# miaoyin390/DNN-Compression-Tensor-ADMM

Measured on AMD Instinct MI355X. Metric: ADMM projection iters/sec (all layers) + per-layer SVD GFLOP/s, ResNet-50 TT ranks, higher is better.
Workload: dtype f32 (Gram, eigen-solve and its filter products accumulate in f64); 1 GPU; resnet50_tt: 34 layers, 20099072 weights, hp table tt_resnet50_hp.HyperParamsDictGeneralRatio3x; tables=1, parallelism=layer-shard x1 (latency-model partition, one scalar all-reduce per step)

## Files before the change

dnn-compression-tensor-admm_amd/csrc/abi_ops.hip:

```cpp
#include "host.h"

using namespace tadmm;

__global__ void square_copy_kernel(const double* __restrict__ in, double* __restrict__ out, int n) {
  const int i = blockIdx.x * blockDim.x + threadIdx.x;
  if (i < n) out[i] = in[i] * in[i];
}

static GemmDesc to_gemm_desc(const tadmm_gemm_desc& s) {
  GemmDesc g;
  memset(&g, 0, sizeof g);
  g.A = s.A; g.B = s.B; g.C = s.C; g.M = s.M; g.N = s.N; g.K = s.K;
  g.a_rs = s.a_rs; g.a_cs = s.a_cs; g.b_rs = s.b_rs; g.b_cs = s.b_cs; g.c_rs = s.c_rs; g.c_cs = s.c_cs;
  g.alpha = s.alpha; g.beta = s.beta; g.bias_n = s.bias_n; g.bias_m = s.bias_m;
  return g;
}

extern "C" {

int tadmm_version(void) { return 100; }

int tadmm_abi_sizes(int* layer_desc_bytes, int* gemm_desc_bytes) {
  if (layer_desc_bytes) *layer_desc_bytes = (int)sizeof(tadmm_layer_desc);
  if (gemm_desc_bytes) *gemm_desc_bytes = (int)sizeof(tadmm_gemm_desc);
// ... 260 lines not shown
  if (c->dtype == TADMM_CHAIN_F16)
    CTX_FAIL(h, TADMM_ERR_INVALID, "conv chain: binary16 is inference only (tadmm_ttconv_fused)");
  ConvChainDesc d;
  const int rc = conv_chain_shape(h, c, mode, d, nullptr);
  if (rc != TADMM_OK) return rc;
  if (r1 <= 0 || r1 > c->R1 || r2 <= 0 || r2 > c->R2)
    CTX_FAIL(h, TADMM_ERR_INVALID, "conv chain: true ranks (%d, %d) outside (0, %d] x (0, %d]", r1, r2, c->R1, c->R2);
  const bool bwd = mode == TADMM_CONV_CHAIN_BWD;
  if (!bwd && (!s1 || !s2) && c->B > 0) CTX_FAIL(h, TADMM_ERR_INVALID, "conv chain: null intermediate (H1, H2)");
  if (bwd && (s1 == nullptr) != (s2 == nullptr)) CTX_FAIL(h, TADMM_ERR_INVALID, "conv chain: dH1 and dH2 are saved together or not at all");
  if (c->B > 0 && (!c->X || !c->Y || !c->W1 || !c->W2 || !c->W3)) CTX_FAIL(h, TADMM_ERR_INVALID, "conv chain: null operand");
  const uintptr_t esz = c->dtype == TADMM_CHAIN_F32 ? 4 : 2;
  if (((uintptr_t)c->X | (uintptr_t)c->Y | (uintptr_t)s1 | (uintptr_t)s2) & (esz - 1))
    CTX_FAIL(h, TADMM_ERR_INVALID, "conv chain: misaligned operand");
  if (!conv_chain_planes_ok(c, d) || (!bwd && (((uintptr_t)c->bias) & 15)))
    CTX_FAIL(h, TADMM_ERR_INVALID, "conv chain: weight planes too small or misaligned");
  if (c->B == 0) return TADMM_OK;
  conv_chain_operands(c, d);
  d.bias = bwd ? nullptr : c->bias;
  d.S1 = bwd ? s2 : s1; d.S2 = bwd ? s1 : s2;
  d.r1t = bwd ? r2 : r1; d.r2t = bwd ? r1 : r2;
  return conv_chain_launch(h, d, c->dtype, (hipStream_t)stream_);
}

int tadmm_ttconv_fused_save(tadmm_handle h, const tadmm_conv_chain_desc* d, int r1, int r2, void* H1, void* H2, void* stream) {
  return conv_chain_train(h, d, TADMM_CONV_CHAIN_FWD, r1, r2, H1, H2, stream);
}

int tadmm_ttconv_fused_bwd(tadmm_handle h, const tadmm_conv_chain_desc* d, int r1, int r2, void* dH1, void* dH2, void* stream) {
  return conv_chain_train(h, d, TADMM_CONV_CHAIN_BWD, r1, r2, dH1, dH2, stream);
}

int tadmm_ttconv_fused_plan(const tadmm_conv_chain_desc* c, int mode, int* tile_pixels, int* tile_rows, int* halo_tiles,
                            int* tiles_per_image, size_t* lds_bytes) {
  if (!c || (mode != TADMM_CONV_CHAIN_FWD && mode != TADMM_CONV_CHAIN_BWD)) return TADMM_ERR_INVALID;
  ConvChainDesc d;
  size_t lds = 0;
  const int rc = conv_chain_shape(nullptr, c, mode, d, &lds);
  if (rc != TADMM_OK) return rc;
  if (tile_pixels) *tile_pixels = d.TM;
  if (tile_rows) *tile_rows = d.TR;
  if (halo_tiles) *halo_tiles = d.NT;
  if (tiles_per_image) *tiles_per_image = d.tiles;
  if (lds_bytes) *lds_bytes = lds;
  return TADMM_OK;
}

int tadmm_core_conv_desc_bytes(void) { return (int)sizeof(tadmm_core_conv_desc); }

int tadmm_core_conv_fwd(tadmm_handle h, const tadmm_core_conv_desc* d, void* stream_) {
  DeviceGuard device_guard(h);
  if (!h) return TADMM_ERR_INVALID;
  return launch_core_conv(h, d, 0, (hipStream_t)stream_);
}

int tadmm_core_conv_dgrad(tadmm_handle h, const tadmm_core_conv_desc* d, void* stream_) {
  DeviceGuard device_guard(h);
  if (!h) return TADMM_ERR_INVALID;
  return launch_core_conv(h, d, 1, (hipStream_t)stream_);
}

static EigGeom gram_geom(int m, int n) { return eig_geom(m, n, 256, false); }

size_t tadmm_gram_scratch_bytes(int m, int n) {
  const EigGeom st = gram_geom(m, n);
  const size_t ntp = (size_t)st.nt * (st.nt + 1) / 2;
  const size_t nblk_p = (size_t)st.ksplit * ntp;
  const size_t nblk_r = ((size_t)st.Npad * st.ld + 1023) / 1024;
  return align_up(st.ksplit * ntp * 1024 * 8, 256) + align_up(sizeof(GramDesc), 256) +
         align_up(nblk_p * sizeof(BlockRef), 256) + align_up(nblk_r * sizeof(BlockRef), 256);
}

int tadmm_gram_ld(int m, int n, int* Npad, int* ld) {
  const EigGeom st = gram_geom(m, n);
  if (Npad) *Npad = st.Npad;
  if (ld) *ld = st.ld;
  return st.N;
}

int tadmm_gram_f64(tadmm_handle h, const float* A, int m, int n, double* G, int ldg, void* scratch, size_t scratch_bytes,
                   void* stream_) {
  DeviceGuard device_guard(h);
  if (!h || !A || !G || !scratch || m <= 0 || n <= 0) return TADMM_ERR_INVALID;
  const EigGeom st = gram_geom(m, n);
  if (ldg != st.ld) CTX_FAIL(h, TADMM_ERR_INVALID, "ldg must be %d (tadmm_gram_ld)", st.ld);
  if (scratch_bytes < tadmm_gram_scratch_bytes(m, n)) CTX_FAIL(h, TADMM_ERR_WORKSPACE, "gram scratch too small");
  hipStream_t s = (hipStream_t)stream_;
  const size_t ntp = (size_t)st.nt * (st.nt + 1) / 2;
  char* base = (char*)scratch;
  size_t off = 0;
  double* partial = (double*)(base + off); off += align_up(st.ksplit * ntp * 1024 * 8, 256);
  GramDesc* gdev = (GramDesc*)(base + off); off += align_up(sizeof(GramDesc), 256);
  std::vector<BlockRef> mp, mr;
  for (int b = 0; b < (int)(st.ksplit * ntp); ++b) mp.push_back(BlockRef{0, b});
  if (st.ksplit > 1)
    for (int b = 0; b < (int)(((size_t)st.Npad * st.ld + 1023) / 1024); ++b) mr.push_back(BlockRef{0, b});
  BlockRef* mpd = (BlockRef*)(base + off); off += align_up(mp.size() * sizeof(BlockRef), 256);
  BlockRef* mrd = (BlockRef*)(base + off);
  GramDesc gd;
  memset(&gd, 0, sizeof gd);
  gd.A = A; gd.m = m; gd.n = n; gd.trans = st.trans; gd.N = st.N; gd.K = st.trans ? m : n; gd.nt = st.nt;
  gd.ksplit = st.ksplit; gd.kchunk = st.kchunk; gd.partial = partial; gd.G = G; gd.Npad = st.Npad; gd.ld = st.ld;
  HIP_OK(h, hipMemcpyAsync(gdev, &gd, sizeof gd, hipMemcpyHostToDevice, s));
  HIP_OK(h, hipMemcpyAsync(mpd, mp.data(), mp.size() * sizeof(BlockRef), hipMemcpyHostToDevice, s));
  HIP_OK(h, hipMemcpyAsync(mrd, mr.data(), mr.size() * sizeof(BlockRef), hipMemcpyHostToDevice, s));
  HIP_OK(h, hipStreamSynchronize(s));
  launch_gram_partial(gdev, mpd, (int)mp.size(), s);
  launch_gram_reduce(gdev, mrd, (int)mr.size(), s);
  HIP_OK(h, hipGetLastError());
  return TADMM_OK;
}

size_t tadmm_eigh_scratch_bytes(int N) {
  const EigGeom g = eig_geom(N, N, 64, true);
  const size_t Npad = g.Npad, ld = g.ld;
  return align_up(Npad * ld * 8, 256) + align_up(sizeof(EigDesc), 256) + 3 * align_up(Npad * sizeof(BlockRef), 256) +
         align_up(Npad * 8, 256) * 2 + align_up(Npad * 4, 256) + 1024 + align_up((Npad / 16) * 256 * 8, 256);
}

static int eigh_leading(tadmm_handle h, const double* G, int N, int r, double* evals_out, double* evecs_out,
                        void* scratch, size_t scratch_bytes, int* sweeps_out, int* route_out, void* stream_) {
  DeviceGuard device_guard(h);
  if (!h || !G || !evals_out || !evecs_out || !scratch || N <= 0 || r < 1 || r > N) return TADMM_ERR_INVALID;
  if (scratch_bytes < tadmm_eigh_scratch_bytes(N)) CTX_FAIL(h, TADMM_ERR_WORKSPACE, "eigh scratch too small");
  hipStream_t s = (hipStream_t)stream_;
  const EigGeom geo = eig_geom(N, N, 64, true);
  const int Npad = geo.Npad, ld = geo.ld;
  char* base = (char*)scratch;
  size_t off = 0;
  auto carve = [&](size_t bytes) { const size_t o = off; off += align_up(bytes, 256); return o; };
  double* XT = (double*)(base + carve((size_t)Npad * ld * 8));
  const size_t o_desc = carve(sizeof(EigDesc));
  EigDesc* edev = (EigDesc*)(base + o_desc);
  EigLayout L;
  Phase* phases[3] = {&L.tick, &L.norm, &L.ext};
  size_t o_map[3];
  for (size_t& o : o_map) o = carve(Npad * sizeof(BlockRef));
  double* lam = (double*)(base + carve((size_t)Npad * 8));
  double* sigma = (double*)(base + carve((size_t)Npad * 8));
  int32_t* order = (int32_t*)(base + carve((size_t)Npad * 4));
  double* offs = (double*)(base + off); off += 64;
  int32_t* done = (int32_t*)(base + off); off += 64;
  double* sblk = (double*)(base + off);
  HIP_OK(h, hipMemsetAsync(XT, 0, (size_t)Npad * ld * 8, s));
  HIP_OK(h, hipMemcpy2DAsync(XT, (size_t)ld * 8, G, (size_t)N * 8, (size_t)N * 8, N, hipMemcpyDeviceToDevice, s));
  std::vector<EigDesc> ev(1);
  EigDesc& e = ev[0];
  memset(&e, 0, sizeof e);
  e.XT = XT; e.N = N; e.Npad = Npad; e.ld = ld; e.nb = geo.nb; e.off = offs; e.done = done; e.lam = lam; e.order = order;
  e.sigma = sigma; e.r = r; e.mode = 2; e.out_a = nullptr; e.out_b = nullptr; e.evec_out = evecs_out;
  e.sblk = sblk;
  EigMaps maps;
  if (const int rc = eig_maps(h, L, ev, false, maps)) return rc;
  const std::vector<BlockRef>* mv[3] = {&maps.tick, &maps.norm, &maps.ext};
  HIP_OK(h, hipMemcpyAsync(edev, &e, sizeof e, hipMemcpyHostToDevice, s));
  for (int i = 0; i < 3; ++i) {
    phases[i]->desc_off = o_desc;
    phases[i]->map_off = o_map[i];
    HIP_OK(h, hipMemcpyAsync(base + o_map[i], mv[i]->data(), mv[i]->size() * sizeof(BlockRef), hipMemcpyHostToDevice, s));
  }
  HIP_OK(h, hipStreamSynchronize(s));
  const bool super = L.kernel == EigTick::SuperPairs;
  const int units = L.players[0];
  const BlockRef* m_tick = (const BlockRef*)(base + L.tick.map_off);
  const double tol = 1e-9;
  int tick = 0, gs = 0;
  bool conv = false;
  if (jacobi_small_fits(Npad) && !(getenv("TADMM_EIGH_TICK") && atoi(getenv("TADMM_EIGH_TICK")))) {
    int32_t* fast = done + 4;
    int* verdict = (int*)(done + 8);
    HIP_OK(h, hipMemsetAsync(done, 0, 64, s));
    const bool direct = eig_small_direct_on();
    if (direct) HIP_OK(h, launch_eig_small_direct(edev, 1, nullptr, fast, verdict, s));
    HIP_OK(h, launch_jacobi_small(edev, 1, Npad, tol, 60, nullptr, verdict, s, false, direct ? fast : nullptr));
    int hv[6] = {0, 0, 0, 0, 0, 0};
    HIP_OK(h, hipMemcpyAsync(hv, done + 4, sizeof hv, hipMemcpyDeviceToHost, s));
    HIP_OK(h, hipStreamSynchronize(s));
    conv = hv[5] != 0;
    gs = hv[0] ? 0 : 1;
    if (sweeps_out) *sweeps_out = gs;
    if (route_out) *route_out = hv[0] ? 0 : 1;
    if (!conv) CTX_FAIL(h, TADMM_ERR_NOCONVERGE, "small eigen-solve did not converge");
  } else {
  if (route_out) *route_out = 2;
  launch_jacobi_init(edev, 1, s);
  double hoff[3];
  int hdone = 0;
  for (; gs < 40 && !conv; ++gs) {
    for (int t = 0; t < units - 1; ++t, ++tick) {
      if (super) {
        HIP_OK(h, launch_jacobi_tick3(edev, m_tick, L.tick.nblocks, tick, tol, ld, s));
      } else {
        HIP_OK(h, launch_jacobi_tick(edev, m_tick, L.tick.nblocks, tick, tol, L.tick_lds, s));
      }
    }
    HIP_OK(h, hipMemcpyAsync(hoff, offs, 24, hipMemcpyDeviceToHost, s));
    HIP_OK(h, hipMemcpyAsync(&hdone, done, 4, hipMemcpyDeviceToHost, s));
    HIP_OK(h, hipStreamSynchronize(s));
    conv = hdone || hoff[gs & 1] < tol;
  }
  if (sweeps_out) *sweeps_out = gs;
  if (getenv("TADMM_STAMPS_DUMP")) { (void)hipStreamSynchronize(s); dump_stamps(); }
  if (!conv) CTX_FAIL(h, TADMM_ERR_NOCONVERGE, "Jacobi did not converge in 40 sweeps");
  }
  L.finalize(base, s, nullptr);
  HIP_OK(h, hipGetLastError());
  hipLaunchKernelGGL(square_copy_kernel, dim3((r + 255) / 256), dim3(256), 0, s, sigma, evals_out, r);
  HIP_OK(h, hipGetLastError());
  return TADMM_OK;
}

int tadmm_eigh_f64(tadmm_handle h, const double* G, int N, double* evals_out, double* evecs_out, void* scratch,
                   size_t scratch_bytes, int* sweeps_out, void* stream_) {
  return eigh_leading(h, G, N, N, evals_out, evecs_out, scratch, scratch_bytes, sweeps_out, nullptr, stream_);
}

int tadmm_eigh_partial_f64(tadmm_handle h, const double* G, int N, int r, double* evals_out, double* evecs_out,
                           void* scratch, size_t scratch_bytes, int* route_out, void* stream_) {
  return eigh_leading(h, G, N, r, evals_out, evecs_out, scratch, scratch_bytes, nullptr, route_out, stream_);
}

size_t tadmm_dgemm_scratch_bytes(int M, int N) {
  return align_up(sizeof(DgemmDesc), 256) + align_up((size_t)(M / 32) * (N / 32) * sizeof(BlockRef), 256);
}

int tadmm_dgemm_f64(tadmm_handle h, const double* A, const double* B, double* C, int M, int N, int K, int lda, int ldb,
                    int ldc, int b_transposed, void* scratch, size_t scratch_bytes, void* stream_) {
  DeviceGuard device_guard(h);
  if (!h || !A || !B || !C || !scratch) return TADMM_ERR_INVALID;
  if (M <= 0 || N <= 0 || K <= 0 || M % 32 || N % 32 || K % 16 || (lda & 1) || (ldb & 1) || (ldc & 1))
    CTX_FAIL(h, TADMM_ERR_INVALID, "tadmm_dgemm_f64: M, N multiples of 32, K of 16, even leading dimensions");
  if (scratch_bytes < tadmm_dgemm_scratch_bytes(M, N)) CTX_FAIL(h, TADMM_ERR_WORKSPACE, "dgemm scratch too small");
  hipStream_t s = (hipStream_t)stream_;
  DgemmDesc g;
  memset(&g, 0, sizeof g);
  g.A = A; g.B = B; g.C = C; g.selA = g.selB = g.selC = g.selP = g.selQ = -1;
  g.M = M; g.N = N; g.K = K; g.lda = lda; g.ldb = ldb; g.ldc = ldc; g.tiles_m = M / 32; g.tiles_n = N / 32;
  std::vector<BlockRef> map;
  for (int b = 0; b < g.tiles_m * g.tiles_n; ++b) map.push_back(BlockRef{0, b});
  DgemmDesc* gd = (DgemmDesc*)scratch;
  BlockRef* md = (BlockRef*)((char*)scratch + align_up(sizeof(DgemmDesc), 256));
  HIP_OK(h, hipMemcpyAsync(gd, &g, sizeof g, hipMemcpyHostToDevice, s));
  HIP_OK(h, hipMemcpyAsync(md, map.data(), map.size() * sizeof(BlockRef), hipMemcpyHostToDevice, s));
  HIP_OK(h, hipStreamSynchronize(s));
  if (b_transposed && K % 32 == 0 && !getenv("TADMM_DGEMM_OLD")) {
    std::vector<BlockRef> m64;
    for (int b = 0; b < ((M + 63) / 64) * ((N + 63) / 64); ++b) m64.push_back(BlockRef{0, b});
    HIP_OK(h, hipMemcpyAsync(md, m64.data(), m64.size() * sizeof(BlockRef), hipMemcpyHostToDevice, s));
    HIP_OK(h, hipStreamSynchronize(s));
    launch_dgemm_nt64(gd, md, (int)m64.size(), s);
  } else {
    launch_dgemm(gd, md, (int)map.size(), b_transposed != 0, s);
  }
  HIP_OK(h, hipGetLastError());
  return TADMM_OK;
}

size_t tadmm_dgemm3_scratch_bytes(int M, int N) {
  const size_t planes = (size_t)3 * (N / 16) * (N / 32) * 512 * 2;
  return align_up(sizeof(DgemmDesc), 256) + align_up(sizeof(GPlaneDesc), 256) + align_up(planes, 256) +
         2 * align_up(((size_t)(M / 32) * ((N + 63) / 64) + (size_t)(N / 16) * (N / 32) / 4 + 8) * sizeof(BlockRef), 256);
}

int tadmm_dgemm3_f64(tadmm_handle h, const double* A, const double* Gm, double* C, int M, int N, int lda, int ldg, int ldc,
                     int repeats, void* scratch, size_t scratch_bytes, void* stream_) {
  DeviceGuard device_guard(h);
  if (!h || !A || !Gm || !C || !scratch) return TADMM_ERR_INVALID;
  if (M <= 0 || N <= 0 || M % 32 || N % 32 || lda < N || ldg < N || ldc < N || (lda & 1) || (ldg & 1) || (ldc & 1))
    CTX_FAIL(h, TADMM_ERR_INVALID, "tadmm_dgemm3_f64: M, N multiples of 32, even leading dimensions >= N");
  if (scratch_bytes < tadmm_dgemm3_scratch_bytes(M, N)) CTX_FAIL(h, TADMM_ERR_WORKSPACE, "dgemm3 scratch too small");
  hipStream_t s = (hipStream_t)stream_;
  char* base = (char*)scratch;
  size_t off = 0;
  auto take = [&](size_t b) { size_t o = off; off += align_up(b, 256); return o; };
  const size_t o_g = take(sizeof(DgemmDesc)), o_p = take(sizeof(GPlaneDesc));
  const int nt = N / 16, ks = N / 32;
  const int64_t plane = (int64_t)nt * ks * 512;
  const size_t o_planes = take((size_t)3 * plane * 2);
  std::vector<BlockRef> m_gp, m_fast;
  for (int b = 0; b < (nt * ks + 3) / 4; ++b) m_gp.push_back(BlockRef{0, b});
  const int tn = (N + 63) / 64;
  for (int b = 0; b < (M / 32) * tn; ++b) m_fast.push_back(BlockRef{0, b});
  xcd_by_key(m_fast, [&](const BlockRef& b) { return b.local % tn; });
  const size_t o_mgp = take(m_gp.size() * sizeof(BlockRef)), o_mf = take(m_fast.size() * sizeof(BlockRef));
  GPlaneDesc gd;
  memset(&gd, 0, sizeof gd);
  gd.Gm = Gm; gd.ldg = ldg; gd.nt = nt; gd.ks = ks; gd.out = (uint16_t*)(base + o_planes); gd.plane = plane;
  DgemmDesc g;
  memset(&g, 0, sizeof g);
  g.A = A; g.C = C; g.selA = g.selB = g.selC = g.selP = g.selQ = -1;
  g.M = M; g.N = N; g.K = N; g.lda = lda; g.ldb = ldg; g.ldc = ldc; g.tiles_m = M / 32; g.tiles_n = N / 32;
  g.Gp = (const uint16_t*)(base + o_planes); g.g_plane = plane;
  HIP_OK(h, hipMemcpyAsync(base + o_g, &g, sizeof g, hipMemcpyHostToDevice, s));
  HIP_OK(h, hipMemcpyAsync(base + o_p, &gd, sizeof gd, hipMemcpyHostToDevice, s));
  HIP_OK(h, hipMemcpyAsync(base + o_mgp, m_gp.data(), m_gp.size() * sizeof(BlockRef), hipMemcpyHostToDevice, s));
  HIP_OK(h, hipMemcpyAsync(base + o_mf, m_fast.data(), m_fast.size() * sizeof(BlockRef), hipMemcpyHostToDevice, s));
  HIP_OK(h, hipStreamSynchronize(s));
  launch_gplanes((const GPlaneDesc*)(base + o_p), (const BlockRef*)(base + o_mgp), (int)m_gp.size(), s);
  for (int i = 0; i < std::max(1, repeats); ++i)
    launch_dgemm3((const DgemmDesc*)(base + o_g), (const BlockRef*)(base + o_mf), (int)m_fast.size(), s);
  HIP_OK(h, hipGetLastError());
  return TADMM_OK;
}

size_t tadmm_cholqr_scratch_bytes(int n, int ncols) {
  return align_up(sizeof(DgemmDesc), 256) + align_up(sizeof(CholDesc), 256) + 2 * align_up((size_t)n * n * 8, 256) +
         align_up((size_t)n * 16 * 8, 256) + align_up((size_t)(n / 32) * (n / 32) * sizeof(BlockRef), 256) +
         align_up((size_t)(ncols / kCholStrip) * sizeof(BlockRef), 256) + 256;
}

int tadmm_cholqr_f64(tadmm_handle h, double* YT, int n, int ncols, int ldy, void* scratch, size_t scratch_bytes,
                     int* bad_out_host, void* stream_) {
  DeviceGuard device_guard(h);
  if (!h || !YT || !scratch || !bad_out_host) return TADMM_ERR_INVALID;
  if (n <= 0 || n > 256 || n % 32 || ncols <= 0 || ncols % 64 || ldy < ncols || (ldy & 1))
    CTX_FAIL(h, TADMM_ERR_INVALID, "tadmm_cholqr_f64: n multiple of 32 (<= 256), ncols multiple of 64, ldy >= ncols even");
  if (scratch_bytes < tadmm_cholqr_scratch_bytes(n, ncols)) CTX_FAIL(h, TADMM_ERR_WORKSPACE, "cholqr scratch too small");
  hipStream_t s = (hipStream_t)stream_;
  char* base = (char*)scratch;
  size_t off = 0;
  DgemmDesc* gd = (DgemmDesc*)(base + off); off += align_up(sizeof(DgemmDesc), 256);
  CholDesc* cd = (CholDesc*)(base + off); off += align_up(sizeof(CholDesc), 256);
  double* Cm = (double*)(base + off); off += align_up((size_t)n * n * 8, 256);
  double* Rm = (double*)(base + off); off += align_up((size_t)n * n * 8, 256);
  double* Wd = (double*)(base + off); off += align_up((size_t)n * 16 * 8, 256);
  BlockRef* mg = (BlockRef*)(base + off); off += align_up((size_t)(n / 32) * (n / 32) * sizeof(BlockRef), 256);
  BlockRef* ms = (BlockRef*)(base + off); off += align_up((size_t)(ncols / kCholStrip) * sizeof(BlockRef), 256);
  int32_t* bad = (int32_t*)(base + off);
  DgemmDesc g;
  memset(&g, 0, sizeof g);
  g.A = YT; g.B = YT; g.C = Cm; g.selA = g.selB = g.selC = g.selP = g.selQ = -1;
  g.M = n; g.N = n; g.K = ncols; g.lda = ldy; g.ldb = ldy; g.ldc = n; g.tiles_m = n / 32; g.tiles_n = n / 32;
  CholDesc c;
  memset(&c, 0, sizeof c);
  c.C = Cm; c.ldc = n; c.n = n; c.R = Rm; c.ldr = n; c.Wd = Wd;
  c.ring[0] = YT; c.ring[1] = YT; c.ring[2] = YT; c.rot = nullptr; c.sel = 0; c.ldy = ldy; c.ncols = ncols; c.bad = bad;
  std::vector<BlockRef> vg, vs;
  for (int b = 0; b < g.tiles_m * g.tiles_n; ++b) vg.push_back(BlockRef{0, b});
  for (int b = 0; b < ncols / kCholStrip; ++b) vs.push_back(BlockRef{0, b});
  HIP_OK(h, hipMemsetAsync(bad, 0, 4, s));
  HIP_OK(h, hipMemcpyAsync(gd, &g, sizeof g, hipMemcpyHostToDevice, s));
  HIP_OK(h, hipMemcpyAsync(cd, &c, sizeof c, hipMemcpyHostToDevice, s));
  HIP_OK(h, hipMemcpyAsync(mg, vg.data(), vg.size() * sizeof(BlockRef), hipMemcpyHostToDevice, s));
  HIP_OK(h, hipMemcpyAsync(ms, vs.data(), vs.size() * sizeof(BlockRef), hipMemcpyHostToDevice, s));
// ... 96 lines not shown
```

dnn-compression-tensor-admm_amd/csrc/common.h:

```cpp
#pragma once
#include <hip/hip_runtime.h>
#include <stdint.h>
#include <stddef.h>
#include "../../include/tadmm.h"

namespace tadmm {

constexpr int kWave = 64;

struct BlockRef { int32_t prob; int32_t local; };

struct SweepDesc {
  const float* W; float* U; float* Z;
  float* T0;
  const float* Zmat;
  int32_t O, I, K2;
  int32_t ichunk;
  int32_t nchunk;
  int64_t numel;
  int32_t blk_begin;
  int32_t nblk;
};

void launch_unfold(const SweepDesc* descs_dev, const BlockRef* map_dev, int nblocks, int use_u, hipStream_t s);
void launch_fold_update(const SweepDesc* descs_dev, const BlockRef* map_dev, int nblocks, int update_u,
                        double* resid_partial_dev, hipStream_t s);
void launch_resid_reduce(const SweepDesc* descs_dev, int nlayers, const double* resid_partial_dev,
                         double* resid_sq_dev, hipStream_t s, const int32_t* out_index = nullptr);

struct GramDesc {
  const float* A;
  int32_t m, n;
  int32_t trans;
  int32_t N, K;
  int32_t nt;
  int32_t ksplit, kchunk;
  double* partial;
  double* G;
  int32_t Npad, ld;
};
void launch_gram_partial(const GramDesc* descs_dev, const BlockRef* map_dev, int nblocks, hipStream_t s,
                         const int32_t* skip = nullptr);
void launch_gram_reduce(const GramDesc* descs_dev, const BlockRef* map_dev, int nblocks, hipStream_t s,
                        const int32_t* skip = nullptr);

constexpr int kJB = 8;
struct EigDesc {
  double* XT;
  int32_t N, Npad, ld, nb;
  double* off;
  int32_t* done;
  double* lam;
  int32_t* order;
  double* sigma;
  int32_t r;
  int32_t mode;
  float* out_a;
  float* out_b;
  double* evec_out;
  double* sblk;
  int32_t ldo;
  double* warm;
  int32_t* warm_ok;
  double* scratch;
  int32_t period;
};
void launch_jacobi_init(const EigDesc* descs_dev, int nprob, hipStream_t s, const int32_t* skip = nullptr,
                        double* prev_dev = nullptr);
void launch_jacobi_conv(const EigDesc* descs_dev, int nprob, int tick, double tol, bool super, double* prev_dev,
                        int* verdict_pinned, hipStream_t s);
constexpr int kJacobiMaxN = 8160;
bool jacobi_size_supported(int n);
size_t jacobi_tick_stream_lds_bytes();
size_t jacobi_tick_lds_bytes(int ld_max);
hipError_t launch_jacobi_tick(const EigDesc* descs_dev, const BlockRef* map_dev, int nblocks, int tick, double tol,
                              size_t lds_bytes, hipStream_t s);
void dump_stamps();
size_t jacobi_tick3_lds_bytes(int ld_max);
bool jacobi_tick3_fits(int ld_max);
hipError_t launch_jacobi_tick3(const EigDesc* descs_dev, const BlockRef* map_dev, int nblocks, int tick, double tol,
                               int ld_max, hipStream_t s);
constexpr int kLdResidentMax = 1152;
static inline int eig_ld(int N) { return (N + 127) / 128 * 128; }
bool jacobi_small_fits(int npad_max);
hipError_t launch_jacobi_small(const EigDesc* descs_dev, int nprob, int npad_max, double tol, int max_sweeps,
                               const int32_t* skip, int* verdict_pinned, hipStream_t s, bool warm,
                               const int32_t* fast_done = nullptr);
bool eig_small_direct_on();
bool eig_mid_direct_on();
bool eig_mid_direct_size(int n);
size_t eig_mid_scratch_bytes(int n);
void launch_eig_mid_direct(const EigDesc* descs_dev, int nprob, int ns, const int32_t* skip, int* verdict_pinned, hipStream_t s);
hipError_t launch_eig_small_direct(const EigDesc* descs_dev, int nprob, const int32_t* skip, int32_t* fast_done_dev,
                                   int* verdict_pinned, hipStream_t s);
void launch_eig_norms(const EigDesc* descs_dev, const BlockRef* map_dev, int nblocks, hipStream_t s,
                      const int32_t* skip = nullptr);
void launch_eig_sort(const EigDesc* descs_dev, int nprob, hipStream_t s, const int32_t* skip = nullptr, int npad_max = 0);
void launch_eig_extract(const EigDesc* descs_dev, const BlockRef* map_dev, int nblocks, hipStream_t s,
                        const int32_t* skip = nullptr);

struct GemmDesc {
  const float* A; const float* B; float* C;
  int32_t M, N, K;
  int64_t a_rs, a_cs, b_rs, b_cs, c_rs, c_cs;
  float alpha, beta;
  const float* bias_n; const float* bias_m;
  int32_t tiles_m, tiles_n;
};
constexpr int kGemmBM = 64, kGemmBN = 64;
void launch_gemm(const GemmDesc* descs_dev, const BlockRef* map_dev, int nblocks, hipStream_t s,
                 const int32_t* skip = nullptr);
void launch_gemm_one(const GemmDesc& d, hipStream_t s);
void launch_gemm_bf16_nt(const void* A, const void* Bt, void* C, int M, int N, int K, int64_t lda, int64_t ldb,
                         int64_t ldc, const float* bias_n, hipStream_t s);

#if defined(__HIP_DEVICE_COMPILE__) || defined(__HIPCC__)
template <typename T> using G = T __attribute__((address_space(1)));
template <typename T> __device__ __forceinline__ G<T>* gp(T* p) { return (G<T>*)p; }
typedef float f4u __attribute__((ext_vector_type(4), aligned(4)));
#endif

struct ChainDesc {
  const void* X; void* Y;
  const uint16_t* Win; const uint16_t* Wout;
  const float* bias;
  int64_t T;
  int32_t Kin, R, Nout;
  int64_t ldx, ldy, win_plane, wout_plane;
  int32_t x_hw, y_hw, x_vec, y_vec, fused;
  long long* stamps;
  void* H;
  int64_t ldh;
  int32_t rt, h_vec;
};
int launch_tt_chain(const ChainDesc& d, int dtype, int tile_tokens, hipStream_t s);
int launch_svdconv_chain(const ChainDesc& d, int dtype, int tile_tokens, hipStream_t s);

struct ConvChainDesc {
  const void* X; void* Y;
  const uint16_t* W1; const uint16_t* W2; const uint16_t* W3;
  const float* bias;
  int64_t w1_plane, w2_plane, w3_plane;
  int32_t B, C, R1, R2, Nout;
  int32_t H, W, Ho, Wo, kh, kw, sh, sw, ph, pw, dh, dw;
  int32_t TM, TR, tiles, NT;
  int32_t x_vec;
  int32_t transposed;
  void* S1; void* S2;
  int32_t r1t, r2t;
};
int launch_tt_conv(const ConvChainDesc& d, int dtype, hipStream_t s);
bool plan_tt_conv(ConvChainDesc& d, int dtype, size_t* lds_bytes);

struct DgemmDesc {
  const double* A; const double* B; const double* C;
  const double* P; const double* Q;
  double* ring[3];
  const int32_t* rot;
  int32_t selA, selB, selC, selP, selQ;
  int32_t M, N, K;
  int32_t lda, ldb, ldc;
  int32_t tiles_m, tiles_n;
  int32_t mode;
  const double* coef;
  const double* theta;
  double* rowpart;
  const int32_t* gate; int32_t gate_min;
  const uint16_t* Gp; int64_t g_plane;
};
void launch_dgemm(const DgemmDesc* descs_dev, const BlockRef* map_dev, int nblocks, bool b_transposed, hipStream_t s);
void launch_dgemm_nt64(const DgemmDesc* descs_dev, const BlockRef* map_dev, int nblocks, hipStream_t s, int tile_n = 64,
                       int tile_m = 64);
void launch_daxpby(const DgemmDesc* descs_dev, const BlockRef* map_dev, int nblocks, hipStream_t s);
struct GPlaneDesc {
  const double* Gm; int32_t ldg;
  int32_t nt, ks;
  uint16_t* out; int64_t plane;
};
void launch_gplanes(const GPlaneDesc* descs_dev, const BlockRef* map_dev, int nblocks, hipStream_t s);
void launch_dgemm3(const DgemmDesc* descs_dev, const BlockRef* map_dev, int nblocks, hipStream_t s);

constexpr int kCholStrip = 16;
struct CholDesc {
  const double* C; int32_t ldc;
  int32_t n;
  double* R; int32_t ldr;
  double* Wd;
  double* ring[3]; const int32_t* rot; int32_t sel;
  int32_t ldy, ncols;
  int32_t* bad;
  const int32_t* gate; int32_t gate_min;
  int32_t* rot_out;
};
void launch_chol_factor(const CholDesc* descs_dev, int nprob, hipStream_t s);
void launch_chol_solve(const CholDesc* descs_dev, const BlockRef* map_dev, int nblocks, hipStream_t s);

struct FiltState {
  int32_t base, res;
  int32_t nsteps;
  int32_t active;
  int32_t alive;
  int32_t bad;
  int32_t stage;
  int32_t products;
  int32_t products_fast;
  int32_t precise_stages;
  double logamp;
  double logamp_precise;
  double coef1[2];
  double coefk[3];
  double b, lr, l1;
  double crit;
  double guard;
  double mom[64 * 5];
  int32_t mom_on;
};
struct FiltProb {
  FiltState* st;
  double* ring[3];
  int32_t N, Npad, rp, r, r32;
  int32_t ldy;
  const double* rqpart; int32_t rq_tiles;
  const double* vpart; int32_t v_tiles;
  const double* lam; const int32_t* order;
  double* sigma;
  double* theta;
  const double* UT;
  int32_t mode, ldo;
  float* out_a; float* out_b;
  int32_t* skip_slot;
  int32_t* fb_skip;
  const double* G; int32_t ldg;
  const double* H; int32_t ldh;
};
// ... 37 lines not shown
```

dnn-compression-tensor-admm_amd/csrc/host.h:

```cpp
#pragma once
#include "common.h"

#include <algorithm>
#include <atomic>
#include <cstdio>
#include <cstdlib>
#include <cstring>
#include <functional>
#include <string>
#include <vector>

struct tadmm_ctx_s {
  int device = 0;
  std::string err;
};

#define CTX_FAIL(h, code, ...)                                   \
  do {                                                           \
    char _b[512];                                                \
    snprintf(_b, sizeof _b, __VA_ARGS__);                        \
    if (h) (h)->err = _b;                                        \
    return (code);                                               \
  } while (0)

#define HIP_OK(h, call)                                                                              \
  do {                                                                                               \
    hipError_t _e = (call);                                                                          \
    if (_e != hipSuccess) CTX_FAIL(h, TADMM_ERR_HIP, "%s failed: %s", #call, hipGetErrorString(_e)); \
  } while (0)

namespace tadmm {

static inline size_t align_up(size_t v, size_t a) { return (v + a - 1) / a * a; }

struct DeviceGuard {
  int prev = -1;
  bool switched = false;
  explicit DeviceGuard(const tadmm_ctx_s* h) {
    if (!h) return;
    if (hipGetDevice(&prev) != hipSuccess) { prev = -1; return; }
    if (prev != h->device) switched = hipSetDevice(h->device) == hipSuccess;
  }
  ~DeviceGuard() { if (switched) (void)hipSetDevice(prev); }
  DeviceGuard(const DeviceGuard&) = delete;
  DeviceGuard& operator=(const DeviceGuard&) = delete;
};

struct DynLdsOptIn {
  std::atomic<bool> done[64] = {};
  template <class K> hipError_t operator()(K kernel, size_t bytes) {
    int dev = 0;
    hipError_t e = hipGetDevice(&dev);
    if (e != hipSuccess) return e;
    std::atomic<bool>& flag = done[dev & 63];
    if (flag.load(std::memory_order_acquire)) return hipSuccess;
    e = hipFuncSetAttribute(reinterpret_cast<const void*>(kernel), hipFuncAttributeMaxDynamicSharedMemorySize, (int)bytes);
    if (e == hipSuccess) flag.store(true, std::memory_order_release);
    else (void)hipGetLastError();
    return e;
  }
};

int core_conv_check(tadmm_ctx_s* h, const tadmm_core_conv_desc* c, bool need_planes, int planes_rows, int planes_cols);
int launch_core_conv(tadmm_ctx_s* h, const tadmm_core_conv_desc* c, int transposed, hipStream_t s);

struct Phase {
  size_t desc_off = 0, map_off = 0;
  int nprob = 0, nblocks = 0;
};

struct Arena {
  size_t off = 0;
  size_t take(size_t bytes, size_t align = 256) {
    off = align_up(off, align);
    const size_t o = off;
    off += bytes;
    return o;
  }
};

struct HostImage {
  std::vector<char> bytes;
  void put(size_t off, const void* src, size_t n) {
    if (!n) return;
    if (bytes.size() < off + n) bytes.resize(off + n);
    memcpy(bytes.data() + off, src, n);
  }
};

static inline void place_phase(Phase& ph, Arena& da, HostImage* img, const void* descs, size_t dbytes, int nprob,
                               const std::vector<BlockRef>& map) {
  ph.nprob = nprob;
  ph.nblocks = (int)map.size();
  ph.desc_off = da.take(std::max<size_t>(dbytes, 16));
  ph.map_off = da.take(std::max<size_t>(map.size() * sizeof(BlockRef), 16));
  if (img) {
    img->put(ph.desc_off, descs, dbytes);
    img->put(ph.map_off, map.data(), map.size() * sizeof(BlockRef));
  }
}

static inline void place_map_like(Phase& ph, const Phase& like, Arena& da, HostImage* img, const std::vector<BlockRef>& map) {
  ph = like;
  ph.nblocks = (int)map.size();
  ph.map_off = da.take(std::max<size_t>(map.size() * sizeof(BlockRef), 16));
  if (img) img->put(ph.map_off, map.data(), map.size() * sizeof(BlockRef));
}

static inline size_t set_gemm_tiles(GemmDesc& g) {
  g.tiles_m = (g.M + kGemmBM - 1) / kGemmBM;
  g.tiles_n = (g.N + kGemmBN - 1) / kGemmBN;
  return (size_t)g.tiles_m * g.tiles_n;
}
static inline void gemm_tiles(GemmDesc& g, int prob, std::vector<BlockRef>& map) {
  const int nt = (int)set_gemm_tiles(g);
  for (int b = 0; b < nt; ++b) map.push_back(BlockRef{prob, b});
}

struct EigGeom {
  int m = 0;
  int64_t cols = 0;
  bool trans = false;
  int N = 0, Npad = 0, nb = 0, ld = 0;
  int nt = 0, ksplit = 1, kchunk = 0;
};

static inline EigGeom eig_geom(int m, int64_t cols, int wg_target, bool cap_chunk) {
  EigGeom g;
  g.m = m; g.cols = cols;
  g.trans = (int64_t)m > cols;
  g.N = (int)std::min<int64_t>(m, cols);
  g.Npad = (int)align_up(g.N, 4 * kJB);
  g.nb = g.Npad / kJB;
  g.ld = eig_ld(g.N);
  g.nt = (g.N + 31) / 32;
  const int64_t K = std::max<int64_t>(1, g.trans ? m : cols);
  const int ntp = std::max(1, g.nt * (g.nt + 1) / 2);
  int ks = (wg_target + ntp - 1) / ntp;
  const int maxks = (int)std::max<int64_t>(1, (K + 255) / 256);
  ks = std::max(1, std::min(ks, maxks));
  if (cap_chunk) ks = std::max(ks, (int)((K + 2047) / 2048));
  g.kchunk = (int)align_up((K + ks - 1) / ks, 64);
  g.ksplit = (int)((K + g.kchunk - 1) / g.kchunk);
  return g;
}

static inline void xcd_group(std::vector<BlockRef>& m) {
  const char* e = getenv("TADMM_XCD_MAP");
  if (e && !atoi(e)) return;
  const int G = (int)m.size();
  if (G < 16) return;
  std::vector<BlockRef> out(G);
  int i = 0;
  for (int x = 0; x < 8; ++x)
    for (int b = x; b < G; b += 8) out[b] = m[i++];
  m.swap(out);
}

static inline void xcd_by_problem(std::vector<BlockRef>& m, const std::vector<double>& weight) {
  const char* e = getenv("TADMM_XCD_MAP");
  if (e && !atoi(e)) return;
  const int G = (int)m.size();
  if (G < 64) return;
  const int np = (int)weight.size();
  std::vector<std::vector<BlockRef>> per(np);
  for (const BlockRef& b : m) per[b.prob].push_back(b);
  std::vector<int> order(np);
  for (int i = 0; i < np; ++i) order[i] = i;
  std::stable_sort(order.begin(), order.end(), [&](int a, int b) {
    return weight[a] * per[a].size() > weight[b] * per[b].size();
  });
  std::vector<std::vector<BlockRef>> bin(8);
  double load[8] = {0};
  for (int p : order) {
    int best = 0;
    for (int x = 1; x < 8; ++x) if (load[x] < load[best]) best = x;
    load[best] += weight[p] * per[p].size();
    bin[best].insert(bin[best].end(), per[p].begin(), per[p].end());
  }
  size_t head[8] = {0};
  std::vector<BlockRef> out;
  out.reserve(G);
  for (int i = 0; (int)out.size() < G; ++i) {
    int x = i & 7;
    if (head[x] >= bin[x].size()) {
      int full = -1; size_t left = 0;
      for (int y = 0; y < 8; ++y) if (bin[y].size() - head[y] > left) { left = bin[y].size() - head[y]; full = y; }
      if (full < 0) break;
      x = full;
    }
    out.push_back(bin[x][head[x]++]);
  }
  m.swap(out);
}

template <class KeyFn>
static inline void xcd_by_key(std::vector<BlockRef>& m, KeyFn key) {
  const char* e = getenv("TADMM_XCD_MAP");
  if (e && !atoi(e)) return;
  const int G = (int)m.size();
  if (G < 64) return;
  std::vector<std::vector<BlockRef>> bin(8);
  for (const BlockRef& b : m) bin[(size_t)(key(b) & 7)].push_back(b);
  size_t head[8] = {0};
  std::vector<BlockRef> out;
  out.reserve(G);
  for (int i = 0; (int)out.size() < G; ++i) {
    int x = i & 7;
    if (head[x] >= bin[x].size()) {
      int full = -1; size_t left = 0;
      for (int y = 0; y < 8; ++y) if (bin[y].size() - head[y] > left) { left = bin[y].size() - head[y]; full = y; }
      if (full < 0) break;
      x = full;
    }
    out.push_back(bin[x][head[x]++]);
  }
  m.swap(out);
}

enum class EigTick {
  Pairs,
  SuperPairs,
};
static inline EigTick choose_eig_tick(int ld_max) {
  const char* em = getenv("TADMM_JACOBI_MODE");
  const bool want_pairs = em && atoi(em) == 0;
  return (!want_pairs && jacobi_tick3_fits(ld_max)) ? EigTick::SuperPairs : EigTick::Pairs;
}

static inline bool align_sweeps_on() {
  static const bool on = !(getenv("TADMM_JACOBI_ALIGN") && !atoi(getenv("TADMM_JACOBI_ALIGN")));
  return on;
}

struct PollCtx {
  hipEvent_t ev[2];
  int* host = nullptr;
  size_t stride = 0;
  bool made = false;
  hipError_t create(size_t max_problems) {
    stride = (max_problems + 1 + 15) & ~(size_t)15;
    hipError_t e = hipHostMalloc((void**)&host, 2 * stride * sizeof(int), hipHostMallocDefault);
    for (int i = 0; i < 2 && e == hipSuccess; ++i) e = hipEventCreateWithFlags(&ev[i], hipEventDisableTiming);
    made = e == hipSuccess;
    return e;
  }
  void destroy() {
    if (!made) return;
    for (auto& e : ev) (void)hipEventDestroy(e);
    (void)hipHostFree(host);
    made = false;
  }
};

struct JacobiTiming {
  bool on = false;
  hipEvent_t a{}, b{};
  double tick_ms = 0.0; int tick_launches = 0; double tick_flops = 0.0; double tick_wgs = 0.0;
  double small_ms = 0.0; int small_launches = 0; double small_flops = 0.0;
  const int* small_n = nullptr;
};

struct EigGroup {
  const EigDesc* ed = nullptr;
  int neig = 0;
  const int* players = nullptr;
  int gsteps = 0;
  EigTick kernel = EigTick::Pairs;
  int ld_max = 0;
  size_t tick_lds = 0;
  const BlockRef* tick_map = nullptr; int tick_blocks = 0;
  double* prev_dev = nullptr;
  const int32_t* skip = nullptr;
  int npad_max = 0;
  int expected = 0;
  bool aligned = false;
  bool warm = false;
  const int* row_len = nullptr;
  const int* mid_sizes = nullptr;
  std::function<void(hipStream_t)> after_init;
  std::function<void(hipStream_t)> behind_last;
  const double* off_dev = nullptr; const int* done_dev = nullptr;
};

struct EigLayout {
  Phase tick, norm, ext;
  std::vector<int> players;
  std::vector<int> row_len;
  std::vector<int> mid;
  int neig = 0;
  int gsteps = 0;
  EigTick kernel = EigTick::Pairs;
  int ld_max = 0, npad_max = 0;
  size_t tick_lds = 0;
  bool aligned = false;
  size_t prev_off = 0;
  int last_sweeps = 0;

  EigGroup group(char* ws, const int32_t* skip) const {
    EigGroup g;
    g.ed = (const EigDesc*)(ws + tick.desc_off); g.neig = neig;
    g.players = players.data(); g.row_len = row_len.data(); g.mid_sizes = mid.data();
    g.gsteps = gsteps; g.kernel = kernel; g.aligned = aligned;
    g.ld_max = ld_max; g.npad_max = npad_max; g.tick_lds = tick_lds;
    g.tick_map = (const BlockRef*)(ws + tick.map_off); g.tick_blocks = tick.nblocks;
    g.prev_dev = (double*)(ws + prev_off);
    g.skip = skip;
    return g;
  }
  void sort(char* ws, hipStream_t s, const int32_t* skip) const {
    const EigDesc* ed = (const EigDesc*)(ws + tick.desc_off);
    launch_eig_norms(ed, (const BlockRef*)(ws + norm.map_off), norm.nblocks, s, skip);
    launch_eig_sort(ed, neig, s, skip, npad_max);
  }
  void extract(char* ws, hipStream_t s, const int32_t* skip) const {
    launch_eig_extract((const EigDesc*)(ws + tick.desc_off), (const BlockRef*)(ws + ext.map_off), ext.nblocks, s, skip);
  }
  void finalize(char* ws, hipStream_t s, const int32_t* skip) const { sort(ws, s, skip); extract(ws, s, skip); }
};

struct EigMaps { std::vector<BlockRef> tick, norm, ext; };
static inline int eig_maps(tadmm_handle h, EigLayout& l, std::vector<EigDesc>& descs, bool align, EigMaps& m) {
  for (const EigDesc& e : descs)
    if (e.ld <= 0 || e.ld % 128)
      CTX_FAIL(h, TADMM_ERR_INVALID, "internal: eigen-problem (N = %d) with rows of %d doubles; the Jacobi kernels need a "
               "multiple of 128", e.N, e.ld);
  l.neig = (int)descs.size();
  l.ld_max = l.npad_max = l.gsteps = 0;
  l.players.clear(); l.row_len.clear(); l.mid.clear();
  for (const EigDesc& e : descs) { l.ld_max = std::max(l.ld_max, e.ld); l.npad_max = std::max(l.npad_max, e.Npad); }
  l.kernel = descs.empty() ? EigTick::Pairs : choose_eig_tick(l.ld_max);
  const bool super = l.kernel == EigTick::SuperPairs;
  l.tick_lds = jacobi_tick_lds_bytes(l.ld_max);
  for (int pq = 0; pq < l.neig; ++pq) {
    const EigDesc& e = descs[pq];
    const int units = super ? e.nb / 2 : e.nb;
    l.players.push_back(units);
    l.row_len.push_back(e.ld);
    l.mid.push_back((e.scratch && eig_mid_direct_size(e.N) && e.N == e.Npad) ? e.N : 0);
    l.gsteps = std::max(l.gsteps, units - 1);
    for (int b = 0; b < units / 2; ++b) m.tick.push_back(BlockRef{pq, b});
    for (int b = 0; b < (e.Npad + 3) / 4; ++b) m.norm.push_back(BlockRef{pq, b});
    for (int b = 0; b < (e.r + 3) / 4; ++b) m.ext.push_back(BlockRef{pq, b});
  }
  xcd_group(m.tick);
  l.aligned = super && align && align_sweeps_on();
  if (l.aligned) for (EigDesc& e : descs) e.period = l.gsteps;
  l.tick.nprob = l.norm.nprob = l.ext.nprob = l.neig;
  l.tick.nblocks = (int)m.tick.size();
  l.norm.nblocks = (int)m.norm.size(); l.ext.nblocks = (int)m.ext.size();
  return TADMM_OK;
}

static inline int build_eig_layout(tadmm_handle h, EigLayout& l, std::vector<EigDesc>& descs, bool align, Arena& da,
                                   HostImage* img) {
  EigMaps m;
  const int rc = eig_maps(h, l, descs, align, m);
  if (rc != TADMM_OK) return rc;
  place_phase(l.tick, da, img, descs.data(), descs.size() * sizeof(EigDesc), l.neig, m.tick);
  place_map_like(l.norm, l.tick, da, img, m.norm);
  place_map_like(l.ext, l.tick, da, img, m.ext);
  return TADMM_OK;
}

static inline int run_eig_group(tadmm_handle h, const EigGroup& g, PollCtx& poll, double tol, int max_sweeps, bool debug,
                                hipStream_t s, int* sweeps_out, bool* small_pending, JacobiTiming* jt = nullptr,
                                bool* behind_last_stands = nullptr) {
  const bool super = g.kernel == EigTick::SuperPairs;
  *sweeps_out = 0;
  *small_pending = false;
  if (behind_last_stands) *behind_last_stands = false;
  bool stands = false;
  if (g.neig == 0) return TADMM_OK;
  {
    const char* e = getenv("TADMM_JACOBI_SMALL");
    if (g.npad_max > 0 && jacobi_small_fits(g.npad_max) && !(e && !atoi(e))) {
      const bool timed = jt && jt->on;
      if (timed) (void)hipEventRecord(jt->a, s);
      int32_t* fast = (g.prev_dev && eig_small_direct_on()) ? reinterpret_cast<int32_t*>(g.prev_dev) : nullptr;
      if (fast) HIP_OK(h, launch_eig_small_direct(g.ed, g.neig, g.skip, fast, poll.host, s));
      HIP_OK(h, launch_jacobi_small(g.ed, g.neig, g.npad_max, tol, std::max(max_sweeps, 60), g.skip, poll.host, s, g.warm, fast));
      if (timed) {
        float ms = 0.f;
        (void)hipEventRecord(jt->b, s);
        (void)hipEventSynchronize(jt->b);
        (void)hipEventElapsedTime(&ms, jt->a, jt->b);
        jt->small_ms += ms; jt->small_launches += 1;
        for (int q = 0; q < g.neig && jt->small_n; ++q) { const double nn = jt->small_n[q]; jt->small_flops += 8.0 * nn * nn * nn; }
      }
      HIP_OK(h, hipEventRecord(poll.ev[0], s));
      *small_pending = true;
      return TADMM_OK;
    }
  }
  launch_jacobi_init(g.ed, g.neig, s, g.skip, g.prev_dev);
  if (g.after_init) g.after_init(s);
  if (g.gsteps == 0) return TADMM_OK;
  bool all_done = false;
  int tick = 0, gs = 0, pending = -1, needed = 0;
  std::vector<char> known_done(g.neig, 0);
  if (super && g.mid_sizes && eig_mid_direct_on()) {
    bool any192 = false, any128 = false;
    for (int q = 0; q < g.neig; ++q) { any192 = any192 || g.mid_sizes[q] == 192; any128 = any128 || g.mid_sizes[q] == 128; }
    if (any192 || any128) {
      for (int q = 0; q <= g.neig; ++q) poll.host[q] = 0;
      if (any192) launch_eig_mid_direct(g.ed, g.neig, 192, g.skip, poll.host, s);
      if (any128) launch_eig_mid_direct(g.ed, g.neig, 128, g.skip, poll.host, s);
      HIP_OK(h, hipEventRecord(poll.ev[0], s));
      if (hipEventSynchronize(poll.ev[0]) != hipSuccess) CTX_FAIL(h, TADMM_ERR_HIP, "poll event failed");
      bool every = true;
      for (int q = 0; q < g.neig; ++q) {
        known_done[q] = poll.host[1 + q] != 0;
        every = every && (known_done[q] || g.players[q] < 2);
      }
      if (getenv("TADMM_MID_DEBUG")) {
        int ok = 0, cand = 0;
        for (int q = 0; q < g.neig; ++q) { ok += known_done[q] ? 1 : 0; cand += g.mid_sizes[q] ? 1 : 0; }
        fprintf(stderr, "[tadmm] direct RR route: %d of %d candidates solved (%d problems in the group)\n", ok, cand, g.neig);
      }
      if (every) { *sweeps_out = 0; return TADMM_OK; }
    }
  }
  std::vector<double> h_off;
  std::vector<int> h_done;
  auto consume = [&]() -> int {
    if (pending < 0) return TADMM_OK;
    if (hipEventSynchronize(poll.ev[pending & 1]) != hipSuccess) return TADMM_ERR_HIP;
    const int* v = poll.host + (size_t)(pending & 1) * poll.stride;
    if (v[0]) { all_done = true; needed = pending + 1; }
    for (int q = 0; q < g.neig; ++q) known_done[q] = v[1 + q] != 0;
    pending = -1;
    return TADMM_OK;
  };
  for (; gs < max_sweeps && !all_done; ++gs) {
    for (int t = 0; t < g.gsteps; ++t, ++tick) {
      if (super) {
        const bool timed = jt && jt->on;
        if (timed) (void)hipEventRecord(jt->a, s);
        HIP_OK(h, launch_jacobi_tick3(g.ed, g.tick_map, g.tick_blocks, tick, tol, g.ld_max, s));
        if (timed) {
          float ms = 0.f;
          (void)hipEventRecord(jt->b, s);
          (void)hipEventSynchronize(jt->b);
          (void)hipEventElapsedTime(&ms, jt->a, jt->b);
          jt->tick_ms += ms; jt->tick_launches += 1;
          for (int q = 0; q < g.neig; ++q) {
            if (known_done[q] || g.players[q] < 2) continue;
            const int own = g.players[q] - 1;
            if (g.aligned && (tick % g.gsteps) >= own) continue;
            const double ld = g.row_len ? g.row_len[q] : g.ld_max;
            jt->tick_flops += 2560.0 * ld * (g.players[q] / 2);
            jt->tick_wgs += g.players[q] / 2;
          }
        }
      } else {
        HIP_OK(h, launch_jacobi_tick(g.ed, g.tick_map, g.tick_blocks, tick, tol, g.tick_lds, s));
      }
    }
    launch_jacobi_conv(g.ed, g.neig, tick, tol, super, g.prev_dev, poll.host + (size_t)(gs & 1) * poll.stride, s);
    {
      const hipError_t le = hipGetLastError();
      if (le != hipSuccess) CTX_FAIL(h, TADMM_ERR_HIP, "Jacobi launch failed: %s", hipGetErrorString(le));
    }
    if (debug && g.off_dev) {
      h_off.resize((size_t)g.neig * 3); h_done.resize(g.neig);
      HIP_OK(h, hipMemcpyAsync(h_off.data(), g.off_dev, (size_t)g.neig * 3 * 8, hipMemcpyDeviceToHost, s));
      HIP_OK(h, hipMemcpyAsync(h_done.data(), g.done_dev, (size_t)g.neig * 4, hipMemcpyDeviceToHost, s));
      HIP_OK(h, hipStreamSynchronize(s));
      double mxo = 0; int nd = 0;
      for (int q = 0; q < g.neig; ++q) {
        const int steps = g.players[q] - 1;
        if (h_done[q]) ++nd;
        if (steps > 0 && tick % steps == 0) mxo = std::max(mxo, h_off[3 * q + ((tick / steps - 1) & 1)]);
      }
      fprintf(stderr, "[tadmm]   sweep %d: max observed off %.3e, done %d/%d\n", gs, mxo, nd, g.neig);
    }
    int rc = consume();
    if (rc != TADMM_OK) CTX_FAIL(h, rc, "poll event failed");
    if (all_done) break;
    static const bool lazy_poll = !(getenv("TADMM_POLL_EVERY_SWEEP") && atoi(getenv("TADMM_POLL_EVERY_SWEEP")));
    if (lazy_poll && !(jt && jt->on) && g.expected > 0 && gs + 3 < g.expected) continue;
    HIP_OK(h, hipEventRecord(poll.ev[gs & 1], s));
    pending = gs;
    if (g.expected > 0 && gs + 1 >= g.expected) {
      if (g.behind_last && behind_last_stands) { g.behind_last(s); stands = true; }
      rc = consume();
      if (rc != TADMM_OK) CTX_FAIL(h, rc, "poll event failed");
      if (!all_done) stands = false;
    }
  }
  if (!all_done) {
    const int rc = consume();
    if (rc != TADMM_OK) CTX_FAIL(h, rc, "poll event failed");
  }
  if (debug) {
    int pmax = 0;
    for (int q = 0; q < g.neig; ++q) pmax = std::max(pmax, g.players[q]);
    fprintf(stderr, "[tadmm] eig group: neig=%d players_max=%d ticks/sweep=%d wgs/tick=%d sweeps=%d ticks=%d kernel=%s\n",
            g.neig, pmax, g.gsteps, g.tick_blocks, all_done ? needed : gs, tick, super ? "super-pairs" : "pairs");
  }
  if (!all_done) CTX_FAIL(h, TADMM_ERR_NOCONVERGE, "Jacobi did not converge in %d sweeps", max_sweeps);
  *sweeps_out = needed;
  if (behind_last_stands) *behind_last_stands = stands;
  return TADMM_OK;
}

static inline int check_small_group(tadmm_handle h, const EigGroup& g, PollCtx& poll) {
  if (hipEventSynchronize(poll.ev[0]) != hipSuccess) CTX_FAIL(h, TADMM_ERR_HIP, "poll event failed");
  for (int q = 0; q < g.neig; ++q)
    if (!poll.host[1 + q]) CTX_FAIL(h, TADMM_ERR_NOCONVERGE, "Jacobi (small problems) did not converge, problem %d", q);
  return TADMM_OK;
}

}
```

dnn-compression-tensor-admm_amd/csrc/jacobi.hip:

```cpp
#include "host.h"
#include <algorithm>
#include <cstdio>

namespace tadmm {

typedef double double4_t __attribute__((ext_vector_type(4)));
typedef double double2_t __attribute__((ext_vector_type(2)));

constexpr int kPair = 2 * kJB;
constexpr int kHP = kPair + 2;

__global__ __launch_bounds__(256) void jacobi_init_kernel(const EigDesc* __restrict__ descs,
                                                          const int32_t* __restrict__ skip, double* __restrict__ prev) {
  const EigDesc d = descs[blockIdx.x];
  if (prev && threadIdx.x == 0) prev[blockIdx.x] = 0.0;
  if (skip && skip[blockIdx.x]) {
    if (threadIdx.x == 0) *d.done = 1;
    return;
  }
  __shared__ double red[4];
  double mx = 0.0;
  for (int j = threadIdx.x; j < d.N; j += 256) mx = fmax(mx, fabs(d.XT[(int64_t)j * d.ld + j]));
#pragma unroll
  for (int o = 32; o > 0; o >>= 1) mx = fmax(mx, __shfl_down(mx, o, 64));
  if ((threadIdx.x & 63) == 0) red[threadIdx.x >> 6] = mx;
  __syncthreads();
  if (threadIdx.x == 0) {
    const double g = fmax(fmax(red[0], red[1]), fmax(red[2], red[3]));
    d.off[0] = 1.0; d.off[1] = 1.0; d.off[2] = g * g;
    *d.done = 0;
  }
}

__device__ __forceinline__ void rr_pair(int nb, int step, int q, int& a, int& b) {
  const int m = nb - 1;
  if (q == 0) { a = m; b = step % m; }
  else { a = (step + q) % m; b = (step - q + m) % m; }
}

__device__ __forceinline__ void wave_lds_fence() { __builtin_amdgcn_fence(__ATOMIC_ACQ_REL, "wavefront"); }

__device__ __forceinline__ void lds_barrier() {
  __builtin_amdgcn_fence(__ATOMIC_RELEASE, "workgroup", "local");
  __builtin_amdgcn_s_barrier();
  __builtin_amdgcn_fence(__ATOMIC_ACQUIRE, "workgroup", "local");
}

struct PairScratch {
  double* red;
  double (*H)[kHP];
  double (*Q)[kHP];
  int* rotated;
};
constexpr int kPairScratchDoubles = 4 * 256 + 2 * kPair * kHP + 2;

__device__ __forceinline__ PairScratch carve_scratch(double* base) {
  PairScratch s;
  s.red = base;
  s.H = reinterpret_cast<double (*)[kHP]>(base + 4 * 256);
  s.Q = s.H + kPair;
  s.rotated = reinterpret_cast<int*>(s.Q + kPair);
  return s;
}

struct GramAcc {
  double4_t acc0 = {0, 0, 0, 0}, acc1 = {0, 0, 0, 0};
  __device__ __forceinline__ void add(const double* __restrict__ row, int i0, int i1, int q) {
    for (int i = i0; i < i1; i += 8) {
      const double2_t v = *reinterpret_cast<const double2_t*>(row + i + 2 * q);
      acc0 = __builtin_amdgcn_mfma_f64_16x16x4f64(v.x, v.x, acc0, 0, 0, 0);
      acc1 = __builtin_amdgcn_mfma_f64_16x16x4f64(v.y, v.y, acc1, 0, 0, 0);
    }
  }
  __device__ __forceinline__ double sum(int e) const { return acc0[e] + acc1[e]; }
  __device__ __forceinline__ void store_partial(double* __restrict__ red_w, int lane) const {
#pragma unroll
    for (int e = 0; e < 4; ++e) red_w[lane * 4 + e] = sum(e);
  }
};

__device__ __forceinline__ void pair_gram_reduce(const PairScratch& S, int t) {
  const int l = t >> 2, reg = t & 3;
  const int hr = (l >> 4) + 4 * reg, hc = l & 15;
  S.H[hr][hc] = (S.red[t] + S.red[256 + t]) + (S.red[512 + t] + S.red[768 + t]);
  S.Q[hr][hc] = (hr == hc) ? 1.0 : 0.0;
}

template <int CTRL>
__device__ __forceinline__ double dpp_mov_f64(double v) {
  const int lo = __builtin_amdgcn_mov_dpp(__double2loint(v), CTRL, 0xf, 0xf, false);
  const int hi = __builtin_amdgcn_mov_dpp(__double2hiint(v), CTRL, 0xf, 0xf, false);
  return __hiloint2double(hi, lo);
}
__device__ __forceinline__ double group8_sum(double v) {
  v += dpp_mov_f64<0xB1>(v);
  v += dpp_mov_f64<0x4E>(v);
  v += dpp_mov_f64<0x141>(v);
  return v;
}

template <int CTRL>
__device__ __forceinline__ float dpp_mov_f32(float v) {
  return __int_as_float(__builtin_amdgcn_mov_dpp(__float_as_int(v), CTRL, 0xf, 0xf, false));
}
__device__ __forceinline__ float wave_max_f32(float v) {
  v = fmaxf(v, dpp_mov_f32<0xB1>(v));
  v = fmaxf(v, dpp_mov_f32<0x4E>(v));
  v = fmaxf(v, dpp_mov_f32<0x141>(v));
  v = fmaxf(v, dpp_mov_f32<0x140>(v));
  const int b = __float_as_int(v);
  const float m0 = __int_as_float(__builtin_amdgcn_readlane(b, 0)), m1 = __int_as_float(__builtin_amdgcn_readlane(b, 16));
  const float m2 = __int_as_float(__builtin_amdgcn_readlane(b, 32)), m3 = __int_as_float(__builtin_amdgcn_readlane(b, 48));
  return fmaxf(fmaxf(m0, m1), fmaxf(m2, m3));
}

#ifdef TADMM_STAMPS
__device__ unsigned long long g_stamps[32];
#define STAMP(i, t0) do { if (blockIdx.x == gridDim.x / 2 && threadIdx.x == 0) g_stamps[i] += clock64() - (t0); } while (0)
#else
#define STAMP(i, t0) do {} while (0)
#endif
template <bool kKeepQt = false, bool kMeasure = true>
__device__ __forceinline__ double pair_inner_solve_fast(const PairScratch& S, int lane, double hmax, double tol,
                                                        bool within, double* __restrict__ hcur_out = nullptr) {
  double (*Hs)[kHP] = S.H;
  double (*Qs)[kHP] = S.Q;
#ifdef TADMM_STAMPS
  const unsigned long long ts = clock64();
#endif
  const double inv_hmax = hmax > 0.0 ? 1.0 / hmax : 1.0;
  double mx = 0.0;
  if (kMeasure) {
    const float wscale = (float)(1e-14 / tol);
    float mxf = 0.0f;
#pragma unroll
    for (int k = 0; k < 4; ++k) {
      const int e = lane * 4 + k;
      const int i = e >> 4, j = e & 15;
      if (i < j) {
        const float ri = (float)(Hs[i][i] * inv_hmax), rj = (float)(Hs[j][j] * inv_hmax);
        const float rmin = fminf(ri, rj);
        if (rmin > 1e-28f) {
          const float hij = fabsf((float)(Hs[i][j] * inv_hmax));
          const float w = fmaxf(1.0f, wscale * __builtin_amdgcn_rsqf(rmin));
          mxf = fmaxf(mxf, hij * __builtin_amdgcn_rsqf(ri) * __builtin_amdgcn_rsqf(rj) * __builtin_amdgcn_rcpf(w));
        }
      }
    }
    mx = (double)wave_max_f32(mxf);
  }
  STAMP(10, ts);
  int did = 0;
  if (!kMeasure || mx > 1e-15) {
    const int g8 = lane >> 3, l8 = lane & 7;
    auto rotation = [&](double a, double b, double g, double& c, double& s, double& t) -> bool {
      if (!(g * g > 1e-36 * fabs(a * b) && fabs(g) > 1e-300)) return false;
      const double zd = b - a, wd = 2.0 * g;
      const int ew = __builtin_amdgcn_frexp_exp(wd);
      const int ex = zd == 0.0 ? ew : max(__builtin_amdgcn_frexp_exp(zd), ew);
      const float zf = (float)__builtin_amdgcn_ldexp(zd, -ex), wf = (float)__builtin_amdgcn_ldexp(wd, -ex);
      const float az = fabsf(zf);
      float tf = wf * __builtin_amdgcn_rcpf(az + __builtin_amdgcn_sqrtf(__builtin_fmaf(az, az, wf * wf)));
      if (zf < 0.0f) tf = -tf;
      t = (double)tf;
      const double x = 1.0 + t * t;
      c = __builtin_amdgcn_rsq(x);
      c = c * (1.5 - 0.5 * x * c * c);
      s = t * c;
      return true;
    };
    {
      const int p = g8;
      if (lane < kPair) Hs[lane][kPair] = Hs[lane][lane];
      wave_lds_fence();
      double2_t* yp = reinterpret_cast<double2_t*>(&Hs[p][2 * l8]);
      double2_t* tp = reinterpret_cast<double2_t*>(&Qs[p][2 * l8]);
      double2_t vp = *yp, up = *tp;
      double a = Hs[p][kPair];
      for (int st = 0; st < kJB; ++st) {
        const int q = kJB + ((g8 + st) & (kJB - 1));
        double2_t* yq = reinterpret_cast<double2_t*>(&Hs[q][2 * l8]);
        double2_t* tq = reinterpret_cast<double2_t*>(&Qs[q][2 * l8]);
        const double2_t vq = *yq, uq = *tq;
        const double b = Hs[q][kPair];
        const double g = group8_sum(vp.x * uq.x + vp.y * uq.y);
        double c, s, t;
        if (rotation(a, b, g, c, s, t)) {
          *yq = double2_t{s * vp.x + c * vq.x, s * vp.y + c * vq.y};
          *tq = double2_t{s * up.x + c * uq.x, s * up.y + c * uq.y};
          vp = double2_t{c * vp.x - s * vq.x, c * vp.y - s * vq.y};
          up = double2_t{c * up.x - s * uq.x, c * up.y - s * uq.y};
          if (l8 == 0) Hs[q][kPair] = b + t * g;
          a -= t * g;
          did = 1;
        }
        wave_lds_fence();
      }
      *yp = vp; *tp = up;
      wave_lds_fence();
    }
    STAMP(11, ts);
    for (int st = 0; within && st < kJB - 1; ++st) {
      int a2, b2;
      rr_pair(kJB, st, g8 & 3, a2, b2);
      const int base = (g8 >> 2) * kJB;
      const int p = base + min(a2, b2), q = base + max(a2, b2);
      double2_t* yp = reinterpret_cast<double2_t*>(&Hs[p][2 * l8]);
      double2_t* yq = reinterpret_cast<double2_t*>(&Hs[q][2 * l8]);
      double2_t* tp = reinterpret_cast<double2_t*>(&Qs[p][2 * l8]);
      double2_t* tq = reinterpret_cast<double2_t*>(&Qs[q][2 * l8]);
      const double2_t vp = *yp, vq = *yq, up = *tp, uq = *tq;
      const double a = group8_sum(vp.x * up.x + vp.y * up.y);
      const double b = group8_sum(vq.x * uq.x + vq.y * uq.y);
      const double g = group8_sum(vp.x * uq.x + vp.y * uq.y);
      double c, s, t;
      if (rotation(a, b, g, c, s, t)) {
        *yp = double2_t{c * vp.x - s * vq.x, c * vp.y - s * vq.y};
        *yq = double2_t{s * vp.x + c * vq.x, s * vp.y + c * vq.y};
        *tp = double2_t{c * up.x - s * uq.x, c * up.y - s * uq.y};
        *tq = double2_t{s * up.x + c * uq.x, s * up.y + c * uq.y};
        did = 1;
      }
      wave_lds_fence();
    }
    did = __any(did);
    if (hcur_out) {
#pragma unroll
      for (int k = 0; k < 4; ++k) {
        const int e = lane * 4 + k;
        const int a = e >> 4, b = e & 15;
        double acc = 0.0;
#pragma unroll
        for (int t = 0; t < kPair; ++t) acc += Hs[a][t] * Qs[b][t];
        hcur_out[e] = acc;
      }
    }
    if (!kKeepQt) {
      double qt[4];
#pragma unroll
      for (int k = 0; k < 4; ++k) { const int e = lane * 4 + k; qt[k] = Qs[e & 15][e >> 4]; }
      wave_lds_fence();
#pragma unroll
      for (int k = 0; k < 4; ++k) { const int e = lane * 4 + k; Qs[e >> 4][e & 15] = qt[k]; }
      wave_lds_fence();
    }
  } else if (hcur_out) {
#pragma unroll
    for (int k = 0; k < 4; ++k) { const int e = lane * 4 + k; hcur_out[e] = Hs[e >> 4][e & 15]; }
  }
  if (lane == 0) *S.rotated = did;
  STAMP(12, ts);
  return mx;
}

constexpr int kSuper = 2 * kPair;

__device__ __forceinline__ int sub_index(int u, int v, int k) { return (k < kJB) ? (u * kJB + k) : (v * kJB + (k - kJB)); }

struct TickPos {
  int sweep, step, steps;
  __device__ __forceinline__ TickPos(int tick, int players, int period) {
    steps = players - 1;
    const int per = period > 0 ? period : steps;
    sweep = tick / per;
    step = tick - sweep * per;
  }
  __device__ __forceinline__ bool retired(const EigDesc& d, double tol, bool leader) const {
    if (*d.done) return true;
    if (step == 0 && sweep > 0 && d.off[(sweep - 1) & 1] < tol) {
      if (leader) *d.done = 1;
      return true;
    }
    return false;
  }
  struct State { int done; double prev, hmax; };
  __device__ __forceinline__ State state(const EigDesc& d) const {
    return State{*gp(d.done), gp(d.off)[(sweep - 1) & 1], gp(d.off)[2]};
  }
  __device__ __forceinline__ bool retired(const EigDesc& d, const State& s, double tol, bool leader) const {
    if (s.done) return true;
    if (step == 0 && sweep > 0 && s.prev < tol) {
      if (leader) *gp(d.done) = 1;
      return true;
    }
    return false;
  }
  __device__ __forceinline__ void record(const EigDesc& d, double mx) const {
    __hip_atomic_fetch_max(gp(reinterpret_cast<unsigned long long*>(&d.off[sweep & 1])),
                           (unsigned long long)__double_as_longlong(mx), __ATOMIC_RELAXED, __HIP_MEMORY_SCOPE_AGENT);
  }
  __device__ __forceinline__ void clear_next(const EigDesc& d, bool leader) const {
    if (step == steps - 1 && leader) gp(d.off)[(sweep + 1) & 1] = 0.0;
  }
};

struct SlabCols {
  double* XT;
  int ld, a, b, half, c0;
  __device__ __forceinline__ int64_t at(int k) const {
    return (int64_t)((k < half) ? (a * half + k) : (b * half + (k - half))) * ld + c0;
  }
};

__device__ __forceinline__ void dma_load_slab(double* Xs, int ldp, const SlabCols& g, int len, int wave, int nwaves,
                                              int lane) {
  const int cpr = len >> 7;
  const int npiece = 2 * g.half * cpr;
  for (int c = wave; c < npiece; c += nwaves) {
    const int row = c / cpr, ch = c - row * cpr;
    const double* src = g.XT + g.at(row) + ch * 128 + lane * 2;
    double* dst = Xs + row * ldp + ch * 128;
    __builtin_amdgcn_global_load_lds((const __attribute__((address_space(1))) void*)src,
                                     (__attribute__((address_space(3))) void*)dst, 16, 0, 0);
  }
}

enum class QDst { Slab, Global, GlobalAgent };
template <bool kQt, QDst kDst>
__device__ __forceinline__ void apply_q_tiles(double* Xs, int ldp, int ncol, const double (*Q)[kHP], int u, int v, int wi,
                                              int nw, int lane, const SlabCols& g = SlabCols{}) {
  const int r = lane & 15, q = lane >> 4;
  double qa[4];
  int rowk[4];
  int64_t growk[4];
#pragma unroll
  for (int t = 0; t < 4; ++t) {
    qa[t] = kQt ? Q[r][4 * t + q] : Q[4 * t + q][r];
    const int row = sub_index(u, v, 4 * t + q);
    rowk[t] = row * ldp;
    growk[t] = (kDst == QDst::Slab) ? 0 : g.at(row);
  }
  G<double>* xt = gp(g.XT);
  const int ntile = ncol >> 4;
  for (int it = wi; it < ntile; it += nw) {
    const int col = it * 16 + r;
    double4_t acc = {0, 0, 0, 0};
#pragma unroll
    for (int t = 0; t < 4; ++t) acc = __builtin_amdgcn_mfma_f64_16x16x4f64(qa[t], Xs[rowk[t] + col], acc, 0, 0, 0);
#pragma unroll
    for (int e = 0; e < 4; ++e) {
      if (kDst == QDst::Slab) Xs[rowk[e] + col] = acc[e];
      else if (kDst == QDst::Global) xt[growk[e] + col] = acc[e];
      else __hip_atomic_store(xt + growk[e] + col, acc[e], __ATOMIC_RELAXED, __HIP_MEMORY_SCOPE_AGENT);
    }
  }
}

__global__ __launch_bounds__(256) void jacobi_tick_kernel(const EigDesc* __restrict__ descs,
                                                          const BlockRef* __restrict__ map, int tick, double tol) {
  extern __shared__ __attribute__((aligned(16))) double smem[];
  const BlockRef br = map[blockIdx.x];
  const EigDesc d = descs[br.prob];
  const TickPos pos(tick, d.nb, 0);
  const int tid = threadIdx.x, lane = tid & 63, wave = tid >> 6;
  const bool leader = br.local == 0 && tid == 0;
  const TickPos::State st = pos.state(d);
  if (pos.retired(d, st, tol, leader)) return;
  const int ld = d.ld, ldp = ld + 2;
  double* Xs = smem;
  const PairScratch S = carve_scratch(Xs + kPair * ldp);

  int ba, bb;
  rr_pair(d.nb, pos.step, br.local, ba, bb);
  const int r = lane & 15, q = lane >> 4;
  const SlabCols cols{d.XT, ld, ba, bb, kJB, 0};

  dma_load_slab(Xs, ldp, cols, ld, wave, 4, lane);
  __builtin_amdgcn_s_waitcnt(0);
  __syncthreads();
  pos.clear_next(d, leader);

  const int per = ld >> 2;
  GramAcc h;
  h.add(Xs + r * ldp, wave * per, (wave + 1) * per, q);
  h.store_partial(S.red + wave * 256, lane);
  __syncthreads();
  pair_gram_reduce(S, tid);
  __syncthreads();
  if (wave == 0) {
    const double mx = pair_inner_solve_fast(S, lane, st.hmax, tol, pos.step == 0);
    if (lane == 0) pos.record(d, mx);
  }
  __syncthreads();
  if (!*S.rotated) return;

  apply_q_tiles<false, QDst::Global>(Xs, ldp, ld, S.Q, 0, 1, wave, 4, lane, cols);
}

constexpr int kStreamChunk = 1024;

__global__ __launch_bounds__(256) void jacobi_tick_stream_kernel(const EigDesc* __restrict__ descs,
                                                                 const BlockRef* __restrict__ map, int tick,
                                                                 double tol) {
  extern __shared__ __attribute__((aligned(16))) double smem[];
  const BlockRef br = map[blockIdx.x];
  const EigDesc d = descs[br.prob];
  const TickPos pos(tick, d.nb, 0);
  const int tid = threadIdx.x, lane = tid & 63, wave = tid >> 6;
  const bool leader = br.local == 0 && tid == 0;
  if (pos.retired(d, tol, leader)) return;
  constexpr int ldp = kStreamChunk + 2;
  const int ld = d.ld;
  double* Xs = smem;
  const PairScratch S = carve_scratch(Xs + kPair * ldp);
  int ba, bb;
  rr_pair(d.nb, pos.step, br.local, ba, bb);
  const int r = lane & 15, q = lane >> 4;
  SlabCols cols{d.XT, ld, ba, bb, kJB, 0};

  GramAcc h;
  for (int c0 = 0; c0 < ld; c0 += kStreamChunk) {
    const int len = min(kStreamChunk, ld - c0);
    if (c0) __syncthreads();
    cols.c0 = c0;
    dma_load_slab(Xs, ldp, cols, len, wave, 4, lane);
    __builtin_amdgcn_s_waitcnt(0);
    __syncthreads();
    const int per = len >> 2;
    h.add(Xs + r * ldp, wave * per, (wave + 1) * per, q);
  }
  h.store_partial(S.red + wave * 256, lane);
  pos.clear_next(d, leader);
  __syncthreads();
  pair_gram_reduce(S, tid);
  __syncthreads();
  if (wave == 0) {
    const double mx = pair_inner_solve_fast(S, lane, d.off[2], tol, pos.step == 0, nullptr);
    if (lane == 0)
      atomicMax(reinterpret_cast<unsigned long long*>(&d.off[pos.sweep & 1]), (unsigned long long)__double_as_longlong(mx));
  }
  __syncthreads();
  if (!*S.rotated) return;

  const int last0 = ((ld - 1) / kStreamChunk) * kStreamChunk;
  for (int c0 = last0; c0 >= 0; c0 -= kStreamChunk) {
    const int len = min(kStreamChunk, ld - c0);
    cols.c0 = c0;
    if (c0 != last0) {
      __syncthreads();
      dma_load_slab(Xs, ldp, cols, len, wave, 4, lane);
      __builtin_amdgcn_s_waitcnt(0);
      __syncthreads();
    }
    apply_q_tiles<false, QDst::Global>(Xs, ldp, len, S.Q, 0, 1, wave, 4, lane, cols);
  }
}

constexpr int kH32 = kSuper + 2;

__device__ __forceinline__ double pair_measure_h32(const double (*H32)[kH32], int u, int v, int lane, double hmax,
                                                   double tol) {
  const double inv_hmax = hmax > 0.0 ? 1.0 / hmax : 1.0;
  const float wscale = (float)(1e-14 / tol);
  float mxf = 0.0f;
#pragma unroll
  for (int k = 0; k < 4; ++k) {
    const int e = lane * 4 + k;
    const int i = e >> 4, j = e & 15;
    if (i < j) {
      const int gi = sub_index(u, v, i), gj = sub_index(u, v, j);
      const float ri = (float)(H32[gi][gi] * inv_hmax), rj = (float)(H32[gj][gj] * inv_hmax);
      const float rmin = fminf(ri, rj);
      if (rmin > 1e-28f) {
        const float hij = fabsf((float)(H32[gi][gj] * inv_hmax));
        const float w = fmaxf(1.0f, wscale * __builtin_amdgcn_rsqf(rmin));
        mxf = fmaxf(mxf, hij * __builtin_amdgcn_rsqf(ri) * __builtin_amdgcn_rsqf(rj) * __builtin_amdgcn_rcpf(w));
      }
    }
  }
  return (double)wave_max_f32(mxf);
}

template <int ua, int va, int ub, int vb, bool kLdsBarriers = false>
__device__ __forceinline__ void transform_h32(double (*H32)[kH32], const double (*Qa)[kHP], const double (*Qb)[kHP],
                                              int tid) {
  const int lane = tid & 63, wave = tid >> 6;
  const int r = lane & 15, kq = lane >> 4;
  const int I = (wave >> 1) & 1, J = wave & 1;
  const double (*QI)[kHP] = I ? Qb : Qa;
  const double (*QJ)[kHP] = J ? Qb : Qa;
  auto idx = [](int blk, int k) { return blk ? sub_index(ub, vb, k) : sub_index(ua, va, k); };
  double4_t acc = {0, 0, 0, 0}, out = {0, 0, 0, 0};
  if (wave < 4) {
#pragma unroll
    for (int t = 0; t < 4; ++t)
      acc = __builtin_amdgcn_mfma_f64_16x16x4f64(H32[idx(I, r)][idx(J, 4 * t + kq)], QJ[r][4 * t + kq], acc, 0, 0, 0);
#pragma unroll
    for (int t = 0; t < 4; ++t) out = __builtin_amdgcn_mfma_f64_16x16x4f64(QI[r][4 * t + kq], acc[t], out, 0, 0, 0);
  }
  if (kLdsBarriers) lds_barrier(); else __syncthreads();
  if (wave < 4) {
#pragma unroll
    for (int e = 0; e < 4; ++e) H32[idx(I, kq + 4 * e)][idx(J, r)] = out[e];
  }
  if (kLdsBarriers) lds_barrier(); else __syncthreads();
}

__global__ __launch_bounds__(512) void jacobi_tick3_kernel(const EigDesc* __restrict__ descs,
                                                           const BlockRef* __restrict__ map, int tick, double tol) {
  extern __shared__ __attribute__((aligned(16))) double smem[];
  const BlockRef br = map[blockIdx.x];
  const EigDesc d = descs[br.prob];
  const TickPos pos(tick, d.nb >> 1, d.period);
  if (pos.step >= pos.steps) return;
  const bool first = pos.step == 0;
  const int tid = threadIdx.x, lane = tid & 63, wave = tid >> 6;
  const int half = wave >> 2, wv = wave & 3, th = tid & 255;
  const bool leader = br.local == 0 && tid == 0;
  const int ld = d.ld, ldp = ld + 2;
#ifdef TADMM_STAMPS
  const unsigned long long t0 = clock64();
  if (blockIdx.x == gridDim.x / 2 && tid == 0) g_stamps[31] += 1;
#endif
  double* Xs = smem;
  double* R = Xs + kSuper * ldp;
  double (*H32)[kH32] = reinterpret_cast<double (*)[kH32]>(R);
  double* hb = R + 2048 + half * (3 * kPair * kHP);
  double (*Hs)[kHP] = reinterpret_cast<double (*)[kHP]>(hb);
  double (*Q1)[kHP] = Hs + kPair;
  double (*Q2)[kHP] = Q1 + kPair;
  double (*Q1o)[kHP] = reinterpret_cast<double (*)[kHP]>(R + 2048 + (1 - half) * (3 * kPair * kHP)) + kPair;
  double (*Q2o)[kHP] = Q1o + kPair;
  int* flags = reinterpret_cast<int*>(R + 2048 + 2 * (3 * kPair * kHP));

  int sa, sb;
  rr_pair(d.nb >> 1, pos.step, br.local, sa, sb);
  const int r = lane & 15, q = lane >> 4;
  const SlabCols cols{d.XT, ld, sa, sb, kPair, 0};
  G<double>* sblk = gp(d.sblk) + (int64_t)(tid < 256 ? sa : sb) * (kPair * kPair) + th;

  dma_load_slab(Xs, ldp, cols, ld, wave, 8, lane);
  const TickPos::State st = pos.state(d);
  double sreg = first ? 0.0 : *sblk;
  __builtin_amdgcn_s_waitcnt(0);
  if (pos.retired(d, st, tol, leader)) return;
  __syncthreads();
  STAMP(0, t0);
  pos.clear_next(d, leader);
  const double hmax = st.hmax;

  if (first) {
    PairScratch S;
    S.red = R + half * 1024; S.H = Hs; S.Q = Q1; S.rotated = flags + 4 + half;
    double* hcur = &Q2[0][0];
    const int per = ld >> 2;
    GramAcc h;
    h.add(Xs + (half * kPair + r) * ldp, wv * per, (wv + 1) * per, q);
    h.store_partial(S.red + wv * 256, lane);
    __syncthreads();
    pair_gram_reduce(S, th);
    __syncthreads();
    if (wv == half) {
      const double mx = pair_inner_solve_fast(S, lane, hmax, tol, true, hcur);
      if (lane == 0) pos.record(d, mx);
    }
    __syncthreads();
    sreg = hcur[th];
    if (flags[4 + half]) apply_q_tiles<false, QDst::Slab>(Xs, ldp, ld, Q1, 2 * half, 2 * half + 1, wv, 4, lane);
    __syncthreads();
    STAMP(6, t0);
  }

  {
    const int per = ld >> 3;
    const double* ra = Xs + r * ldp + 2 * q;
    const double* rb = Xs + (kPair + r) * ldp + 2 * q;
    double4_t acc0 = {0, 0, 0, 0}, acc1 = {0, 0, 0, 0};
    for (int i = wave * per; i < (wave + 1) * per; i += 8) {
      const double2_t va = *reinterpret_cast<const double2_t*>(ra + i);
      const double2_t vb = *reinterpret_cast<const double2_t*>(rb + i);
      acc0 = __builtin_amdgcn_mfma_f64_16x16x4f64(va.x, vb.x, acc0, 0, 0, 0);
      acc1 = __builtin_amdgcn_mfma_f64_16x16x4f64(va.y, vb.y, acc1, 0, 0, 0);
    }
#pragma unroll
    for (int e = 0; e < 4; ++e) R[wave * 256 + lane * 4 + e] = acc0[e] + acc1[e];
  }
  __syncthreads();
  double cval = 0.0;
  if (tid < 256) {
#pragma unroll
    for (int w = 0; w < 8; ++w) cval += R[w * 256 + tid];
  }
  __syncthreads();
  if (tid < 256) {
    const int l = tid >> 2, reg = tid & 3;
    const int hr = (l >> 4) + 4 * reg, hc = l & 15;
    H32[hr][kPair + hc] = cval;
    H32[kPair + hc][hr] = cval;
    H32[th >> 4][th & 15] = sreg;
  } else {
    H32[kPair + (th >> 4)][kPair + (th & 15)] = sreg;
  }
  __syncthreads();
  STAMP(1, t0);

  double mxall = 0.0;
  const int mwave = (half + 2) & 3;
  {
    const int u = half ? 1 : 0, v = half ? 3 : 2;
    Hs[th >> 4][th & 15] = H32[sub_index(u, v, th >> 4)][sub_index(u, v, th & 15)];
    Q1[th >> 4][th & 15] = ((th >> 4) == (th & 15)) ? 1.0 : 0.0;
    __syncthreads();
    if (wv == half) {
      PairScratch S;
      S.H = Hs; S.Q = Q1; S.rotated = flags + half;
      pair_inner_solve_fast<true, false>(S, lane, hmax, tol, false);
    } else if (wv == mwave) {
      mxall = pair_measure_h32(H32, u, v, lane, hmax, tol);
    }
    __syncthreads();
  }
  STAMP(2, t0);
  {
    double (*Qa)[kHP] = half ? Q1o : Q1;
    double (*Qb)[kHP] = half ? Q1 : Q1o;
    transform_h32<0, 2, 1, 3>(H32, Qa, Qb, tid);
    const int u = half ? 1 : 0, v = half ? 2 : 3;
    Hs[th >> 4][th & 15] = H32[sub_index(u, v, th >> 4)][sub_index(u, v, th & 15)];
    Q2[th >> 4][th & 15] = ((th >> 4) == (th & 15)) ? 1.0 : 0.0;
    __syncthreads();
  }
  STAMP(3, t0);
  if (wv == half) {
    PairScratch S;
    S.H = Hs; S.Q = Q2; S.rotated = flags + 2 + half;
    __builtin_amdgcn_s_setprio(3);
    pair_inner_solve_fast<true, false>(S, lane, hmax, tol, false);
    __builtin_amdgcn_s_setprio(0);
  } else {
    if (wv == mwave) mxall = fmax(mxall, pair_measure_h32(H32, half ? 1 : 0, half ? 2 : 3, lane, hmax, tol));
    const int u = half ? 1 : 0, v = half ? 3 : 2;
    const int wi = (wv > half) ? wv - 1 : wv;
    if (flags[half]) apply_q_tiles<true, QDst::Slab>(Xs, ldp, ld, Q1, u, v, wi, 3, lane);
  }
  __syncthreads();
  STAMP(4, t0);
  if (wv == mwave && lane == 0) pos.record(d, mxall);
  const int any_rot = flags[0] | flags[1] | flags[2] | flags[3] | (first ? flags[4] | flags[5] : 0);
  if (!any_rot) {
    if (first) *sblk = sreg;
    return;
  }
  {
    const int u = half ? 1 : 0, v = half ? 2 : 3;
    apply_q_tiles<true, QDst::GlobalAgent>(Xs, ldp, ld, Q2, u, v, wv, 4, lane, cols);
  }
  STAMP(5, t0);
  {
    double (*Qa)[kHP] = half ? Q2o : Q2;
    double (*Qb)[kHP] = half ? Q2 : Q2o;
    transform_h32<0, 3, 1, 2, true>(H32, Qa, Qb, tid);
  }
  *sblk = (tid < 256) ? H32[th >> 4][th & 15] : H32[kPair + (th >> 4)][kPair + (th & 15)];
  STAMP(20, t0);
}

constexpr int kSmallNpad = 64;
constexpr int kSmallWaveScratch = 2 * kPair * kHP;

__global__ __launch_bounds__(256) void jacobi_small_kernel(const EigDesc* __restrict__ descs,
                                                           const int32_t* __restrict__ skip, double tol,
                                                           int max_sweeps, int* __restrict__ verdict,
                                                           const int32_t* __restrict__ fast_done) {
  extern __shared__ __attribute__((aligned(16))) double smem[];
  const int p = blockIdx.x;
  if (fast_done && fast_done[p]) return;
  const EigDesc d = descs[p];
  const int tid = threadIdx.x, lane = tid & 63, wave = tid >> 6;
  if (skip && skip[p]) {
    if (tid == 0) { *d.done = 1; verdict[1 + p] = 1; }
    return;
  }
  const int Npad = d.Npad, ld = d.ld, ldp = Npad + 2, nb = d.nb;
  const int pairs = nb >> 1, steps = nb - 1;
  double* Xs = smem;
  double* wbase = Xs + Npad * ldp + wave * kSmallWaveScratch;
  double (*Hs)[kHP] = reinterpret_cast<double (*)[kHP]>(wbase);
  double (*Qs)[kHP] = Hs + kPair;
  double* red = Xs + Npad * ldp + 4 * kSmallWaveScratch;
  int* flags = reinterpret_cast<int*>(red + 8);
  double* __restrict__ XT = d.XT;
  {
    const int c2n = Npad >> 1;
    for (int idx = tid; idx < Npad * c2n; idx += 256) {
      const int row = idx / c2n, c2 = idx - row * c2n;
      *reinterpret_cast<double2_t*>(Xs + row * ldp + 2 * c2) =
          *reinterpret_cast<const double2_t*>(XT + (int64_t)row * ld + 2 * c2);
    }
// ... 66 lines not shown
  {
    const int c2n = Npad >> 1;
    for (int idx = tid; idx < Npad * c2n; idx += 256) {
      const int row = idx / c2n, c2 = idx - row * c2n;
      *reinterpret_cast<double2_t*>(XT + (int64_t)row * ld + 2 * c2) =
          *reinterpret_cast<const double2_t*>(Xs + row * ldp + 2 * c2);
    }
  }
  if (d.warm) {
    __shared__ int warm_bad;
    if (tid == 0) warm_bad = conv ? 0 : 1;
    __syncthreads();
    const double floor2 = 1e-16 * hmax;
    for (int jrow = wave; jrow < Npad; jrow += 4) {
      const double* row = Xs + jrow * ldp;
      double s = 0.0;
      for (int i = lane; i < Npad; i += 64) s += row[i] * row[i];
#pragma unroll
      for (int o = 32; o > 0; o >>= 1) s += __shfl_xor(s, o, 64);
      double inv = 0.0;
      if (jrow < d.N) {
        if (s > floor2 && s > 0.0) inv = 1.0 / sqrt(s);
        else if (lane == 0) warm_bad = 1;
      }
      for (int i = lane; i < Npad; i += 64) d.warm[(int64_t)jrow * Npad + i] = row[i] * inv;
    }
    __syncthreads();
    if (tid == 0) *d.warm_ok = warm_bad ? 0 : 1;
  }
  if (tid == 0) {
    *d.done = conv ? 1 : 0;
    d.off[0] = m; d.off[1] = (double)sweep; d.off[2] = hmax;
    verdict[1 + p] = conv ? 1 : 0;
  }
}

bool jacobi_small_fits(int npad_max) { return npad_max <= kSmallNpad; }

hipError_t launch_jacobi_small(const EigDesc* descs_dev, int nprob, int npad_max, double tol, int max_sweeps,
                               const int32_t* skip, int* verdict_pinned, hipStream_t s, bool warm, const int32_t* fast_done) {
  if (nprob <= 0) return hipSuccess;
  const size_t lds = ((size_t)npad_max * (npad_max + 2) * (warm ? 2 : 1) + 4 * kSmallWaveScratch + 16) * 8;
  if (lds > 64 * 1024) {
    static DynLdsOptIn allow_lds;
    const hipError_t e = allow_lds(jacobi_small_kernel, 160 * 1024 - 256);
    if (e != hipSuccess) return e;
  }
  hipLaunchKernelGGL(jacobi_small_kernel, dim3(nprob), dim3(256), lds, s, descs_dev, skip, tol, max_sweeps,
                     verdict_pinned, fast_done);
  return hipSuccess;
}

#ifdef TADMM_STAMPS
void dump_stamps() {
  unsigned long long h[32];
  if (hipMemcpyFromSymbol(h, HIP_SYMBOL(g_stamps), sizeof h) != hipSuccess) return;
  const double n = h[31] ? (double)h[31] : 1.0;
  fprintf(stderr, "[stampsS] per launch (2 solves): preamble=%.0f loop=%.0f epilogue=%.0f\n", h[10] / n, (h[11] - h[10]) / n,
          (h[12] - h[11]) / n);
  fprintf(stderr, "[stamps3] launches=%llu cumulative: load=%.0f self(sum/launches)=%.0f gram=%.0f solve1=%.0f xform=%.0f solve2||apply1=%.0f apply2=%.0f end=%.0f\n",
          h[31], h[0] / n, h[6] / n, h[1] / n, h[2] / n, h[3] / n, h[4] / n, h[5] / n, h[20] / n);
}
#else
void dump_stamps() {}
#endif

__global__ __launch_bounds__(256) void eig_norms_kernel(const EigDesc* __restrict__ descs,
                                                        const BlockRef* __restrict__ map,
                                                        const int32_t* __restrict__ skip) {
  const BlockRef br = map[blockIdx.x];
  if (skip && skip[br.prob]) return;
  const EigDesc d = descs[br.prob];
  const int lane = threadIdx.x & 63, wave = threadIdx.x >> 6;
  const int j = br.local * 4 + wave;
  if (j >= d.Npad) return;
  double s = 0.0;
  if (j < d.N) {
    const double* row = d.XT + (int64_t)j * d.ld;
    for (int i = lane; i < d.N; i += 64) s += row[i] * row[i];
#pragma unroll
    for (int o = 32; o > 0; o >>= 1) s += __shfl_down(s, o, 64);
  }
  if (lane == 0) d.lam[j] = (j < d.N) ? sqrt(s) : -1.0;
}

__global__ __launch_bounds__(256) void eig_sort_kernel(const EigDesc* __restrict__ descs,
                                                       const int32_t* __restrict__ skip) {
  extern __shared__ double slam[];
  if (skip && skip[blockIdx.x]) return;
  const EigDesc d = descs[blockIdx.x];
  for (int j = threadIdx.x; j < d.Npad; j += 256) slam[j] = d.lam[j];
  __syncthreads();
  for (int j = threadIdx.x; j < d.Npad; j += 256) {
    const double lj = slam[j];
    int rank = 0;
    for (int i = 0; i < d.Npad; ++i) {
      const double li = slam[i];
      rank += (li > lj) || (li == lj && i < j);
    }
    d.order[rank] = j;
    if (rank < d.r) d.sigma[rank] = sqrt(fmax(lj, 0.0));
  }
}

#ifndef TADMM_RESIDUE_CUT
#define TADMM_RESIDUE_CUT 1e-12
#endif
constexpr double kResidueCut = TADMM_RESIDUE_CUT;
__global__ __launch_bounds__(256) void eig_extract_kernel(const EigDesc* __restrict__ descs,
                                                          const BlockRef* __restrict__ map,
                                                          const int32_t* __restrict__ skip) {
  const BlockRef br = map[blockIdx.x];
  if (skip && skip[br.prob]) return;
  const EigDesc d = descs[br.prob];
  const int lane = threadIdx.x & 63, wave = threadIdx.x >> 6;
  const int c = br.local * 4 + wave;
  if (c >= d.r) return;
  const int j = d.order[c];
  double lam = d.lam[j];
  if (lam <= kResidueCut * d.lam[d.order[0]]) lam = 0.0;
  const double* row = d.XT + (int64_t)j * d.ld;
  double best = -1.0; int besti = 0;
  for (int i = lane; i < d.N; i += 64) {
    const double a = fabs(row[i]);
    if (a > best) { best = a; besti = i; }
  }
#pragma unroll
  for (int o = 32; o > 0; o >>= 1) {
    const double ob = __shfl_down(best, o, 64);
    const int oi = __shfl_down(besti, o, 64);
    if (ob > best || (ob == best && oi < besti)) { best = ob; besti = oi; }
  }
  besti = __shfl(besti, 0, 64);
  const double sgn = (row[besti] < 0.0) ? -1.0 : 1.0;
  const double inv = (lam > 0.0) ? sgn / lam : 0.0;
  const double sig = sqrt(fmax(lam, 0.0));
  const double isig = (sig > 0.0) ? 1.0 / sig : 0.0;
  const int r = d.ldo ? d.ldo : d.r, N = d.N;
  for (int i = lane; i < N; i += 64) {
    const double v = row[i] * inv;
    if (d.mode == 0) {
      d.out_a[(int64_t)i * r + c] = (float)v;
    } else if (d.mode == 1) {
      d.out_a[(int64_t)i * r + c] = (float)(v * isig);
      d.out_b[(int64_t)c * N + i] = (float)(v * sig);
    } else if (d.mode == 3) {
      d.out_a[(int64_t)i * r + c] = (float)(v * isig);
    }
    if (d.evec_out) d.evec_out[(int64_t)c * N + i] = v;
  }
}

__global__ __launch_bounds__(256) void jacobi_conv_kernel(const EigDesc* __restrict__ descs, int nprob, int tick,
                                                          double tol, int super, double* __restrict__ prev,
                                                          int* __restrict__ verdict) {
  __shared__ int open_problems;
  if (threadIdx.x == 0) open_problems = 0;
  __syncthreads();
  for (int q = threadIdx.x; q < nprob; q += 256) {
    const EigDesc d = descs[q];
    if (*d.done) { verdict[1 + q] = 1; continue; }
    const int own = (super ? (d.nb >> 1) : d.nb) - 1;
    const int steps = (own > 0 && d.period > 0) ? d.period : own;
    bool conv = false;
    if (steps > 0 && tick % steps == 0) {
      const int swp = tick / steps - 1;
      const double m = d.off[swp & 1];
      conv = m < tol;
      const double mp = prev[q];
      if (!conv && mp > 0.0 && mp < 1e-1 && m < 1e-3) {
        const double C = 10.0 * fmax(1.0, m / (mp * mp));
        conv = C * m * m < 10.0 * tol;
      }
      prev[q] = m;
    }
    if (conv) *d.done = 1;
    else open_problems = 1;
    verdict[1 + q] = conv ? 1 : 0;
  }
  __syncthreads();
  if (threadIdx.x == 0) verdict[0] = open_problems ? 0 : 1;
}

void launch_jacobi_conv(const EigDesc* descs_dev, int nprob, int tick, double tol, bool super, double* prev_dev,
                        int* verdict_pinned, hipStream_t s) {
  if (nprob <= 0) return;
  hipLaunchKernelGGL(jacobi_conv_kernel, dim3(1), dim3(256), 0, s, descs_dev, nprob, tick, tol, super ? 1 : 0, prev_dev,
                     verdict_pinned);
}

void launch_jacobi_init(const EigDesc* descs_dev, int nprob, hipStream_t s, const int32_t* skip, double* prev_dev) {
  if (nprob <= 0) return;
  hipLaunchKernelGGL(jacobi_init_kernel, dim3(nprob), dim3(256), 0, s, descs_dev, skip, prev_dev);
}

size_t jacobi_tick_stream_lds_bytes() { return ((size_t)kPair * (kStreamChunk + 2) + kPairScratchDoubles) * 8; }
bool jacobi_size_supported(int n) { return n >= 1 && n <= kJacobiMaxN; }
size_t jacobi_tick_lds_bytes(int ld_max) { return ((size_t)kPair * (ld_max + 2) + kPairScratchDoubles) * 8; }
size_t jacobi_tick3_lds_bytes(int ld_max) {
  return ((size_t)kSuper * (ld_max + 2) + 2048 + 2 * (3 * kPair * kHP)) * 8 + 32;
}
bool jacobi_tick3_fits(int ld_max) { return jacobi_tick3_lds_bytes(ld_max) <= 160 * 1024; }
hipError_t launch_jacobi_tick3(const EigDesc* descs_dev, const BlockRef* map_dev, int nblocks, int tick, double tol,
                               int ld_max, hipStream_t s) {
  if (nblocks <= 0) return hipSuccess;
  static DynLdsOptIn allow_lds;
  hipError_t e = allow_lds(jacobi_tick3_kernel, 160 * 1024);
  if (e != hipSuccess) return e;
  hipLaunchKernelGGL(jacobi_tick3_kernel, dim3(nblocks), dim3(512), jacobi_tick3_lds_bytes(ld_max), s, descs_dev, map_dev,
                     tick, tol);
  e = hipPeekAtLastError();
  if (e != hipSuccess)
    fprintf(stderr, "[tadmm] jacobi tick3 launch failed: %s (blocks=%d lds=%zu)\n", hipGetErrorString(e), nblocks,
            jacobi_tick3_lds_bytes(ld_max));
  return hipSuccess;
}

hipError_t launch_jacobi_tick(const EigDesc* descs_dev, const BlockRef* map_dev, int nblocks, int tick, double tol,
                              size_t lds_bytes, hipStream_t s) {
  if (nblocks <= 0) return hipSuccess;
  hipError_t e;
  if (lds_bytes > 160 * 1024) {
    static DynLdsOptIn allow_lds;
    if ((e = allow_lds(jacobi_tick_stream_kernel, 160 * 1024)) != hipSuccess) return e;
    hipLaunchKernelGGL(jacobi_tick_stream_kernel, dim3(nblocks), dim3(256), jacobi_tick_stream_lds_bytes(), s, descs_dev,
                       map_dev, tick, tol);
  } else {
    static DynLdsOptIn allow_tick_lds;
    if ((e = allow_tick_lds(jacobi_tick_kernel, 160 * 1024)) != hipSuccess) return e;
    hipLaunchKernelGGL(jacobi_tick_kernel, dim3(nblocks), dim3(256), lds_bytes, s, descs_dev, map_dev, tick, tol);
  }
  e = hipPeekAtLastError();
  if (e != hipSuccess)
    fprintf(stderr, "[tadmm] jacobi tick launch failed: %s (blocks=%d lds=%zu)\n", hipGetErrorString(e), nblocks,
            lds_bytes);
  return hipSuccess;
}
void launch_eig_norms(const EigDesc* descs_dev, const BlockRef* map_dev, int nblocks, hipStream_t s,
                      const int32_t* skip) {
  if (nblocks <= 0) return;
  hipLaunchKernelGGL(eig_norms_kernel, dim3(nblocks), dim3(256), 0, s, descs_dev, map_dev, skip);
}
void launch_eig_sort(const EigDesc* descs_dev, int nprob, hipStream_t s, const int32_t* skip, int npad_max) {
  if (nprob <= 0) return;
  hipLaunchKernelGGL(eig_sort_kernel, dim3(nprob), dim3(256), (size_t)std::max(2048, (npad_max > 0 && npad_max <= kJacobiMaxN) ? npad_max : kJacobiMaxN) * 8, s, descs_dev, skip);
}
void launch_eig_extract(const EigDesc* descs_dev, const BlockRef* map_dev, int nblocks, hipStream_t s,
                        const int32_t* skip) {
  if (nblocks <= 0) return;
  hipLaunchKernelGGL(eig_extract_kernel, dim3(nblocks), dim3(256), 0, s, descs_dev, map_dev, skip);
}

}
```

dnn-compression-tensor-admm_amd/csrc/plan.hip:

```cpp
#include "host.h"
#include "filter_host.h"

#include <cmath>
#include <condition_variable>
#include <mutex>
#include <thread>

using namespace tadmm;

struct StepGeom : EigGeom {
  StepGeom() = default;
  explicit StepGeom(const EigGeom& g) : EigGeom(g) {}
  int r = 0;
  bool skip = false;
};

struct LayerGeom {
  tadmm_layer_desc desc;
  int64_t numel = 0;
  int O = 0, I = 0, K2 = 1;
  int d = 0;
  std::vector<StepGeom> steps;
};

// ... 113 lines not shown
  JacobiTiming jtm;
  const int32_t* resid_index = nullptr;
  struct Lanes* lanes = nullptr;
};

struct Lanes {
  tadmm_plan_s* sub[2] = {nullptr, nullptr};
  std::vector<int> lane_of, local_of;
  hipStream_t st[2] = {nullptr, nullptr};
  hipEvent_t ev_begin = nullptr, ev_end[2] = {nullptr, nullptr};
  std::thread worker;
  std::mutex mu;
  std::condition_variable cv;
  int job = 0;
  bool done = true;
  int a_update_u = 0, a_use_u = 0;
  double* a_resid = nullptr;
  int rc = 0;
};

namespace {

struct Built {
  std::vector<size_t> tbuf0, tbuf1, xt, gpart, vs, cores_ws;
};

}

static int layout_plan(tadmm_plan_s* P, const float* const* W, float* const* U, float* const* Z, float* const* cores,
                       HostImage* img, size_t desc_region, size_t* desc_bytes, size_t* total_bytes) {
  tadmm_handle h = P->h;
  const int n = P->n;
  Arena da;
  Arena ar;
  ar.off = desc_region;
  auto dev = [&](size_t off) -> char* { return P->ws ? P->ws + off : nullptr; };

  std::vector<size_t> tb0(n), tb1(n), xt(n), gp(n), vs(n), cw(n);
  std::vector<std::vector<size_t>> core_off(n);
  std::vector<std::vector<float*>> core_ptr(n);
  P->sigma_off.assign(n, {});
  for (int l = 0; l < n; ++l) {
    const LayerGeom& g = P->layers[l];
    tb0[l] = ar.take((size_t)g.numel * 4);
    tb1[l] = ar.take((size_t)g.numel * 4);
    size_t xtb = 0, gpb = 0, vsb = 0, cb = 0;
    for (const StepGeom& st : g.steps) {
      if (st.skip) continue;
      xtb = std::max(xtb, (size_t)st.Npad * st.ld * 8);
      gpb = std::max(gpb, (size_t)st.ksplit * (st.nt * (st.nt + 1) / 2) * 1024 * 8);
      if (st.trans) vsb = std::max(vsb, (size_t)st.N * st.r * 4);
      cb += align_up((size_t)st.m * st.r * 4, 256);
    }
    xt[l] = ar.take(xtb ? xtb : 256);
    gp[l] = ar.take(gpb ? gpb : 256);
    vs[l] = ar.take(vsb ? vsb : 256);
    cw[l] = ar.take(cb ? cb : 256);
    P->sigma_off[l].assign(g.steps.size(), (size_t)-1);
  }

  std::vector<SweepDesc> sd(n);
  std::vector<BlockRef> smap;
  std::vector<float*> cur(n), other(n);
  for (int l = 0; l < n; ++l) {
    const LayerGeom& g = P->layers[l];
    SweepDesc& s = sd[l];
    memset(&s, 0, sizeof s);
    s.W = W ? W[l] : nullptr; s.U = U ? U[l] : nullptr; s.Z = Z ? Z[l] : nullptr;
    s.T0 = (float*)dev(tb0[l]);
    s.O = g.O; s.I = g.I; s.K2 = g.K2;
    s.numel = g.numel;
    if (g.K2 > 1) {
      int ich = std::min(g.I, 512);
      while ((int64_t)g.K2 * (ich + 4) > 12288 && ich > 1) ich /= 2;
      s.ichunk = ich;
      s.nchunk = (g.I + ich - 1) / ich;
      s.nblk = g.O * s.nchunk;
    } else {
      s.ichunk = 8192;
      s.nchunk = (int)((g.numel + s.ichunk - 1) / s.ichunk);
      s.nblk = s.nchunk;
    }
    s.blk_begin = (int)smap.size();
    for (int b = 0; b < s.nblk; ++b) smap.push_back(BlockRef{l, b});
    cur[l] = (float*)dev(tb0[l]);
    other[l] = (float*)dev(tb1[l]);
  }
  P->total_sweep_blocks = (int)smap.size();
  P->resid_partial_off = ar.take((size_t)smap.size() * 8);

  int maxsteps = 0;
  for (const LayerGeom& g : P->layers) maxsteps = std::max(maxsteps, (int)g.steps.size());
  std::vector<int> lvl_off(n, 0);
  {
    std::vector<int> lvl_nb(maxsteps, 0);
    std::vector<long> lvl_wgs(maxsteps, 0);
    std::vector<int> order(n);
    for (int l = 0; l < n; ++l) order[l] = l;
    auto heavy = [&](int l) { int m = 0; for (const StepGeom& st : P->layers[l].steps) if (!st.skip) m = std::max(m, st.nb); return m; };
    std::stable_sort(order.begin(), order.end(), [&](int a, int b) {
      const size_t ca = P->layers[a].steps.size(), cb = P->layers[b].steps.size();
      if (ca != cb) return ca > cb;
      return heavy(a) > heavy(b);
    });
    for (int l : order) {
      const LayerGeom& g = P->layers[l];
      const int len = (int)g.steps.size();
      int best = 0; double best_cost = 1e300;
      for (int off = 0; off + len <= maxsteps; ++off) {
        double cost = 0;
        for (int s = 0; s < len; ++s) {
          if (g.steps[s].skip) continue;
          const int lv = off + s;
          cost += 1e6 * std::max(0, g.steps[s].nb - lvl_nb[lv]) + (double)lvl_wgs[lv] * g.steps[s].nb;
        }
        if (cost < best_cost) { best_cost = cost; best = off; }
      }
      lvl_off[l] = best;
      for (int s = 0; s < len; ++s) {
        if (g.steps[s].skip) continue;
        lvl_nb[best + s] = std::max(lvl_nb[best + s], g.steps[s].nb);
        lvl_wgs[best + s] += g.steps[s].nb / 2;
      }
    }
  }
  P->steps.assign(maxsteps, StepPlan());
  struct RecOp { const float* core; int m, r; int64_t cols; };
  std::vector<std::vector<RecOp>> recops(n);
  std::vector<const float*> lastT(n, nullptr);

  for (int lev = 0; lev < maxsteps; ++lev) {
    StepPlan& sp = P->steps[lev];
    std::vector<GramDesc> gd;
    std::vector<EigDesc> ed;
    std::vector<GemmDesc> pd;
    std::vector<BlockRef> m_gp, m_gr, m_proj;
    std::vector<int> gp_cost;
    std::vector<int> layer_of;
    for (int l = 0; l < n; ++l) {
      const LayerGeom& g = P->layers[l];
      const int s = lev - lvl_off[l];
      if (s < 0 || s >= (int)g.steps.size()) continue;
      const StepGeom& st = g.steps[s];
      if (st.skip) {
        if (cores && cores[l]) CTX_FAIL(h, TADMM_ERR_INVALID, "TADMM_FLAG_SKIP_ROTATIONS is incompatible with cores output");
        continue;
      }
      layer_of.push_back(l);
    }
    const int neig = (int)layer_of.size();
    sp.layer_of = layer_of;
    sp.off_off = ar.take((size_t)std::max(1, neig) * 3 * 8);
    sp.done_off = ar.take((size_t)std::max(1, neig) * 4);
    sp.main.prev_off = ar.take((size_t)std::max(1, neig) * 8);
    sp.skip_off = ar.take((size_t)std::max(1, neig) * 4);
    std::vector<FilterSpec> fspecs;
    sp.filt_of.clear();
    for (int p = 0; p < neig; ++p) {
      const int l = layer_of[p];
      const LayerGeom& g = P->layers[l];
      const int s = lev - lvl_off[l];
      const StepGeom& st = g.steps[s];
      const bool last_step = (s + 2 == g.d);
      float* core_dev;
      float* tnext;
      if (cores && cores[l]) {
        size_t off = 0;
        for (int j = 0; j < s; ++j) off += (size_t)g.steps[j].m * g.steps[j].r;
        core_dev = cores[l] + off;
        tnext = last_step ? (cores[l] + off + (size_t)st.m * st.r) : other[l];
      } else {
        size_t off = 0;
        for (int j = 0; j < s; ++j) if (!g.steps[j].skip) off += align_up((size_t)g.steps[j].m * g.steps[j].r * 4, 256);
        core_dev = (float*)dev(cw[l] + off);
        tnext = other[l];
      }
      const float* Tin = cur[l];
      GramDesc gdsc;
      memset(&gdsc, 0, sizeof gdsc);
      gdsc.A = Tin; gdsc.m = st.m; gdsc.n = (int)st.cols; gdsc.trans = st.trans ? 1 : 0;
      gdsc.N = st.N; gdsc.K = st.trans ? st.m : (int)st.cols;
      gdsc.nt = st.nt; gdsc.ksplit = st.ksplit; gdsc.kchunk = st.kchunk;
      gdsc.partial = (double*)dev(gp[l]);
      gdsc.G = (double*)dev(xt[l]);
      gdsc.Npad = st.Npad; gdsc.ld = st.ld;
      const int ntp = st.nt * (st.nt + 1) / 2;
      for (int b = 0; b < st.ksplit * ntp; ++b) m_gp.push_back(BlockRef{p, b});
      gp_cost.push_back(st.kchunk);
      const int64_t gtot = (int64_t)st.Npad * st.ld;
      if (st.ksplit > 1)
        for (int b = 0; b < (int)((gtot + 1023) / 1024); ++b) m_gr.push_back(BlockRef{p, b});
      gd.push_back(gdsc);
      EigDesc e;
      memset(&e, 0, sizeof e);
      e.XT = (double*)dev(xt[l]);
      e.N = st.N; e.Npad = st.Npad; e.ld = st.ld; e.nb = st.nb;
      e.off = (double*)dev(sp.off_off) + 3 * p;
      e.done = (int32_t*)dev(sp.done_off) + p;
      const size_t lam_off = ar.take((size_t)st.Npad * 8);
      const size_t ord_off = ar.take((size_t)st.Npad * 4);
      const size_t sig_off = ar.take((size_t)st.r * 8);
      const size_t sblk_off = ar.take((size_t)(st.Npad / 16) * 256 * 8);
      P->sigma_off[l][s] = sig_off;
      e.lam = (double*)dev(lam_off);
      e.order = (int32_t*)dev(ord_off);
      e.sigma = (double*)dev(sig_off);
      e.r = st.r;
      e.mode = st.trans ? 1 : 0;
      e.out_a = st.trans ? (float*)dev(vs[l]) : core_dev;
      e.out_b = st.trans ? tnext : nullptr;
      e.evec_out = nullptr;
      e.sblk = (double*)dev(sblk_off);
      ed.push_back(e);
      const bool zonly = (g.desc.flags & TADMM_FLAG_SKIP_ROTATIONS) && !(cores && cores[l]);
      if (const int rp = filter_block_size(st.N, st.r)) {
        FilterSpec fs;
        fs.N = st.N; fs.Npad = st.Npad; fs.ldg = st.ld; fs.r = st.r; fs.rp = rp;
        fs.G = e.XT; fs.mode = e.mode; fs.ldo = e.ldo; fs.out_a = e.out_a; fs.out_b = e.out_b; fs.sigma = e.sigma;
        fs.skip_slot = (int32_t*)dev(sp.skip_off) + p;
        fspecs.push_back(fs);
        sp.filt_of.push_back(p);
      } else if (const int rpc = complement_block_size(st.N, st.r, st.trans, zonly)) {
        FilterSpec fs;
        const int kdis = st.N - st.r;
        fs.N = st.N; fs.Npad = st.Npad; fs.ldg = st.ld; fs.r = kdis; fs.rp = rpc;
        fs.G = (const double*)dev(ar.take((size_t)st.Npad * st.ld * 8));
        fs.g_orig = e.XT; fs.comp_r = st.r; fs.sigma_layer = e.sigma;
        fs.mode = 4; fs.ldo = e.ldo; fs.out_a = e.out_a; fs.out_b = nullptr;
        fs.sigma = (double*)dev(ar.take((size_t)align_up(kdis, 32) * 8));
        fs.skip_slot = (int32_t*)dev(sp.skip_off) + p;
        fspecs.push_back(fs);
        sp.filt_of.push_back(p);
      }
      GemmDesc pg;
      memset(&pg, 0, sizeof pg);
      pg.alpha = 1.f; pg.beta = 0.f;
      if (!st.trans) {
        pg.A = core_dev; pg.a_rs = 1; pg.a_cs = st.r;
        pg.B = Tin; pg.b_rs = st.cols; pg.b_cs = 1;
        pg.C = tnext; pg.c_rs = st.cols; pg.c_cs = 1;
        pg.M = st.r; pg.N = (int)st.cols; pg.K = st.m;
      } else {
        pg.A = Tin; pg.a_rs = st.cols; pg.a_cs = 1;
        pg.B = (const float*)dev(vs[l]); pg.b_rs = st.r; pg.b_cs = 1;
        pg.C = core_dev; pg.c_rs = st.r; pg.c_cs = 1;
        pg.M = st.m; pg.N = st.r; pg.K = (int)st.cols;
      }
      gemm_tiles(pg, p, m_proj);
      pd.push_back(pg);
      recops[l].push_back(RecOp{core_dev, st.m, st.r, st.cols});
      if (tnext == other[l]) std::swap(cur[l], other[l]);
      else { cur[l] = tnext; }
    }
    std::stable_sort(m_gp.begin(), m_gp.end(),
                     [&](const BlockRef& a, const BlockRef& b) { return gp_cost[a.prob] > gp_cost[b.prob]; });
    place_phase(sp.gram_p, da, img, gd.data(), gd.size() * sizeof(GramDesc), neig, m_gp);
    place_map_like(sp.gram_r, sp.gram_p, da, img, m_gr);
    std::vector<EigDesc> ed_fb;
    {
      const int nf = (int)fspecs.size();
      sp.fb_skip_off = ar.take((size_t)std::max(1, nf) * 4);
      for (int i = 0; i < nf; ++i) fspecs[i].fb_skip = (int32_t*)dev(sp.fb_skip_off) + i;
      std::vector<FilterRR> rr;
      filter_layout(sp.fg, fspecs, da, ar, dev, img, rr);
      for (int i = 0; i < nf; ++i) {
        const int p = sp.filt_of[i];
        ed_fb.push_back(ed[p]);
        ed_fb.back().off = (double*)dev(ar.take(3 * 8));
        ed_fb.back().done = (int32_t*)dev(ar.take(4));
        EigDesc e = rr[i].desc;
        e.off = ed[p].off; e.done = ed[p].done;
        ed[p] = e;
      }
    }
    if (const int rc = build_eig_layout(h, sp.main, ed, true, da, img)) return rc;
    sp.fb.prev_off = ar.take((size_t)std::max<size_t>(1, ed_fb.size()) * 8);
    if (const int rc = build_eig_layout(h, sp.fb, ed_fb, true, da, img)) return rc;
    place_phase(sp.proj, da, img, pd.data(), pd.size() * sizeof(GemmDesc), neig, m_proj);
    sp.proj_repeatable = !pd.empty();
    for (const GemmDesc& g : pd) sp.proj_repeatable = sp.proj_repeatable && gemm_repeatable(g);
  }

  for (int l = 0; l < n; ++l) lastT[l] = cur[l];
  size_t maxchain = 0;
  for (int l = 0; l < n; ++l) maxchain = std::max(maxchain, recops[l].size());
  P->recon.assign(maxchain, Phase());
  std::vector<const float*> rcur(n);
  std::vector<float*> rfree(n);
  for (int l = 0; l < n; ++l) {
    rcur[l] = lastT[l];
    float* b0 = (float*)dev(tb0[l]);
    float* b1 = (float*)dev(tb1[l]);
    rfree[l] = (rcur[l] == b0) ? b1 : b0;
  }
  for (size_t lev = 0; lev < maxchain; ++lev) {
    std::vector<GemmDesc> rd;
    std::vector<BlockRef> rmap;
    for (int l = 0; l < n; ++l) {
      if (lev >= recops[l].size()) continue;
      const RecOp& op = recops[l][recops[l].size() - 1 - lev];
      GemmDesc g;
      memset(&g, 0, sizeof g);
      g.alpha = 1.f;
      g.A = op.core; g.a_rs = op.r; g.a_cs = 1;
      g.B = rcur[l]; g.b_rs = op.cols; g.b_cs = 1;
      g.C = rfree[l]; g.c_rs = op.cols; g.c_cs = 1;
      g.M = op.m; g.N = (int)op.cols; g.K = op.r;
      gemm_tiles(g, (int)rd.size(), rmap);
      rd.push_back(g);
      float* b0 = (float*)dev(tb0[l]);
      float* b1 = (float*)dev(tb1[l]);
      const float* produced = rfree[l];
      rfree[l] = (produced == b0) ? b1 : b0;
      rcur[l] = produced;
    }
    place_phase(P->recon[lev], da, img, rd.data(), rd.size() * sizeof(GemmDesc), (int)rd.size(), rmap);
  }
  for (int l = 0; l < n; ++l) sd[l].Zmat = rcur[l];

  P->sweep_desc_off = da.take(sd.size() * sizeof(SweepDesc));
  P->unfold.desc_off = P->sweep_desc_off;
  P->unfold.nprob = n;
  P->unfold.nblocks = (int)smap.size();
  P->unfold.map_off = da.take(smap.size() * sizeof(BlockRef));
  P->fold = P->unfold;
  if (img) {
    img->put(P->sweep_desc_off, sd.data(), sd.size() * sizeof(SweepDesc));
    img->put(P->unfold.map_off, smap.data(), smap.size() * sizeof(BlockRef));
  }
  *desc_bytes = align_up(da.off, 4096);
  *total_bytes = align_up(ar.off, 256);
  return TADMM_OK;
}

template <class T, class Get>
static bool sum_over_lanes(tadmm_plan p, T out[4], Get get, bool last_is_max = false) {
  if (!p->lanes) return false;
  T a[4], b[4];
  get(p->lanes->sub[0], a);
  get(p->lanes->sub[1], b);
  for (int i = 0; i < 4; ++i) out[i] = a[i] + b[i];
  if (last_is_max) out[3] = std::max(a[3], b[3]);
  return true;
}

extern "C" {

int tadmm_tt_clamp_ranks(tadmm_layer_desc* desc) {
  if (!desc || desc->d < 2 || desc->d > TADMM_MAX_MODES) return TADMM_ERR_INVALID;
  return clamp_ranks(desc);
}

static int single_workspace_bytes(tadmm_handle h, int n_layers, const tadmm_layer_desc* descs, size_t* bytes) {
  if (!h || !descs || !bytes || n_layers <= 0) return TADMM_ERR_INVALID;
  tadmm_plan_s P;
  P.h = h;
  P.n = n_layers;
  P.layers.resize(n_layers);
  for (int l = 0; l < n_layers; ++l) {
    int rc = build_geom(h, descs[l], P.layers[l]);
    if (rc) return rc;
  }
  P.ws = nullptr;
  size_t db = 0, data = 0;
  int rc = layout_plan(&P, nullptr, nullptr, nullptr, nullptr, nullptr, 0, &db, &data);
  if (rc) return rc;
  *bytes = db + data + 4096;
  return TADMM_OK;
}

static int single_create(tadmm_handle h, int n_layers, const tadmm_layer_desc* descs, const float* const* W,
                         float* const* U, float* const* Z, float* const* cores, void* workspace, size_t workspace_bytes,
                         tadmm_plan* out) {
  DeviceGuard device_guard(h);
  if (!h || !descs || !W || !U || !Z || !workspace || !out || n_layers <= 0) return TADMM_ERR_INVALID;
  tadmm_plan_s* P = new tadmm_plan_s();
  P->h = h;
  P->n = n_layers;
  P->layers.resize(n_layers);
  for (int l = 0; l < n_layers; ++l) {
    int rc = build_geom(h, descs[l], P->layers[l]);
    if (rc) { delete P; return rc; }
  }
  P->ws = (char*)workspace;
  P->ws_bytes = workspace_bytes;
  HostImage img;
  size_t need = 0, db = 0, data0 = 0;
  int rc = layout_plan(P, W, U, Z, cores, nullptr, 0, &db, &data0);
  if (rc) { delete P; return rc; }
  rc = layout_plan(P, W, U, Z, cores, &img, db, &db, &need);
  if (rc) { delete P; return rc; }
  if (need > workspace_bytes) {
    delete P;
    CTX_FAIL(h, TADMM_ERR_WORKSPACE, "workspace too small: need %zu bytes, got %zu", need, workspace_bytes);
  }
  if (!img.bytes.empty()) {
    hipError_t e = hipMemcpy(P->ws, img.bytes.data(), img.bytes.size(), hipMemcpyHostToDevice);
    if (e != hipSuccess) { delete P; CTX_FAIL(h, TADMM_ERR_HIP, "descriptor upload failed: %s", hipGetErrorString(e)); }
  }
  for (const StepPlan& sp : P->steps) {
    hipError_t e = hipSuccess;
    if (sp.fg.zero_bytes) e = hipMemset(P->ws + sp.fg.zero_off, 0, sp.fg.zero_bytes);
    if (e == hipSuccess) e = hipMemset(P->ws + sp.skip_off, 0, (size_t)std::max(1, sp.main.neig) * 4);
    if (e == hipSuccess) e = hipMemset(P->ws + sp.fb_skip_off, 0, (size_t)std::max(1, sp.fg.nf) * 4);
    if (e != hipSuccess) { delete P; CTX_FAIL(h, TADMM_ERR_HIP, "workspace clear failed: %s", hipGetErrorString(e)); }
  }
  if (const char* e = getenv("TADMM_JACOBI_TOL")) P->tol = atof(e);
  if (getenv("TADMM_DEBUG")) P->debug = true;
  size_t maxe = 1;
  for (const StepPlan& sp : P->steps) maxe = std::max<size_t>(maxe, sp.main.neig);
  {
    const hipError_t e = P->poll.create(maxe);
    if (e != hipSuccess) { delete P; CTX_FAIL(h, TADMM_ERR_HIP, "poll buffers: %s", hipGetErrorString(e)); }
  }
  *out = P;
  return TADMM_OK;
}

static int single_run(tadmm_plan p, int update_u, int use_u, double* resid_sq_dev, void* stream_);

static double step_latency_us_full_or_filtered(int N, int r) {
  const int npad = (int)align_up(N, 32);
  if (npad <= 64) return 100.0;
  const int rp = filter_block_size(N, r);
  if (rp) return 7.0 * (8 * 35.0 + 170.0) + (rp / 16 - 1) * 7.0 * (9.0 + 0.02 * (double)align_up(rp, 128));
  return (npad / 16 - 1) * 11.0 * (9.0 + 0.02 * (double)align_up(N, 128));
}

static bool lane_split(tadmm_handle h, int n, const tadmm_layer_desc* descs, std::vector<int>& lane_of) {
// ... 459 lines not shown
```

dnn-compression-tensor-admm_amd/csrc/tucker_plan.hip:

```cpp
#include "host.h"

#include <cmath>

using namespace tadmm;

namespace {

struct OpGeom : EigGeom {
  int r_eff = 0;
  OpGeom() = default;
  OpGeom(int m, int n, int r) : EigGeom(eig_geom(m, n, 64, true)), r_eff(std::min(r, N)) {}
};

struct BigWarm {
  int layer = 0, Npad = 0, ld = 0, nblocks = 0;
  bool apply = true;
  size_t V = 0, Gt = 0, XT = 0, ok = 0;
  size_t desc_off = 0, map_off = 0;
};

struct Lsv {
  std::vector<BigWarm> big;
  Phase gram_p, gram_r, xg;
  EigLayout eig;
// ... 38 lines not shown
    for (int64_t j = (n4 << 2) + threadIdx.x; j < n; j += 256) { const double v = x[j]; acc += v * v; }
  } else {
    for (int64_t i = threadIdx.x; i < n; i += 256) { const double v = x[i]; acc += v * v; }
  }
  red[threadIdx.x] = acc;
  __syncthreads();
  for (int o = 128; o > 0; o >>= 1) {
    if ((int)threadIdx.x < o) red[threadIdx.x] += red[threadIdx.x + o];
    __syncthreads();
  }
  if (threadIdx.x == 0) out[l] = red[0];
}

__global__ __launch_bounds__(256) void bigwarm_check_kernel(const EigDesc* __restrict__ descs, int prob,
                                                            const int32_t* __restrict__ skip, int32_t* __restrict__ ok) {
  if (skip && skip[prob]) return;
  const EigDesc d = descs[prob];
  __shared__ int bad;
  if (threadIdx.x == 0) bad = *d.done ? 0 : 1;
  __syncthreads();
  const double floor_ = 1e-8 * d.lam[d.order[0]];
  int b = 0;
  for (int j = threadIdx.x; j < d.N; j += 256) b |= !(d.lam[j] > floor_ && d.lam[j] > 0.0);
  if (b) bad = 1;
  __syncthreads();
  if (threadIdx.x == 0) *ok = bad ? 0 : 1;
}
__global__ __launch_bounds__(256) void bigwarm_save_kernel(const EigDesc* __restrict__ descs, int prob,
                                                           const int32_t* __restrict__ skip,
                                                           const int32_t* __restrict__ ok, double* __restrict__ V) {
  if ((skip && skip[prob]) || !*ok) return;
  const EigDesc d = descs[prob];
  const int lane = threadIdx.x & 63, j = blockIdx.x * 4 + (threadIdx.x >> 6);
  if (j >= d.Npad) return;
  const double inv = j < d.N ? 1.0 / d.lam[j] : 0.0;
  const double* __restrict__ x = d.XT + (int64_t)j * d.ld;
  double* __restrict__ v = V + (int64_t)j * d.ld;
  for (int i = lane; i < d.ld; i += 64) v[i] = x[i] * inv;
}

__global__ __launch_bounds__(256) void hooi_conv_kernel(int n, int it, const float* __restrict__ tol,
                                                        const double* __restrict__ nT, const double* __restrict__ nC,
                                                        double* __restrict__ err, int32_t* __restrict__ skip,
                                                        int32_t* __restrict__ iters, int* __restrict__ verdict) {
  __shared__ int open_layers;
  if (threadIdx.x == 0) open_layers = 0;
  __syncthreads();
  for (int l = threadIdx.x; l < n; l += 256) {
    if (skip[l]) { verdict[1 + l] = 1; continue; }
    const double t = nT[l];
    const double e = t > 0.0 ? sqrt(fabs(t - nC[l])) / sqrt(t) : 0.0;
    const double prev = err[((it + 1) & 1) * n + l];
    err[(it & 1) * n + l] = e;
    iters[l] = it + 1;
    const bool conv = it > 1 && fabs(e - prev) < (double)tol[l];
    if (conv) skip[l] = 1;
    else open_layers = 1;
    verdict[1 + l] = conv ? 1 : 0;
  }
  __syncthreads();
  if (threadIdx.x == 0) verdict[0] = open_layers ? 0 : 1;
}

}

struct tadmm_tucker_plan_s {
  tadmm_handle h = nullptr;
  int n = 0;
  std::vector<tadmm_layer_desc> descs;
  std::vector<TLayer> L;
  char* ws = nullptr;
  size_t ws_bytes = 0, desc_bytes = 0;
  Lsv lsv[4];
  Phase gemm[5];
  Phase unfold, fold;
  size_t sweep_desc_off = 0, resid_partial_off = 0, fac_begin = 0, fac_end = 0;
  size_t warm_ok_off = 0;
  size_t off_off = 0, done_off = 0, prev_off = 0, skip_off = 0, nT_off = 0, nC_off = 0, err_off = 0, iters_off = 0,
         tol_off = 0, ptrT_off = 0, ptrC_off = 0, numT_off = 0, numC_off = 0;
  PollCtx poll;
  PollCtx hooi;
  double jtol = 1e-9;
  int max_sweeps = 40, n_iter_max = 100;
  bool debug = false;
  int last_hooi = 0, last_jacobi_sweeps = 0;
  JacobiTiming jtm;
  bool ev_made = false;
  hipEvent_t tev[4];
  double last_total_ms = 0.0;
};

static bool warm_start_on() {
  const char* e = getenv("TADMM_TUCKER_WARM");
  return !(e && !atoi(e));
}

static int tucker_layout(tadmm_tucker_plan_s* P, char* base, const float* const* W, float* const* U, float* const* Z,
                         HostImage* img, size_t desc_region, size_t* desc_bytes, size_t* total_bytes) {
  tadmm_handle h = P->h;
  const int n = P->n;
  Arena da, ar;
  ar.off = desc_region;
  auto dev = [&](size_t off) -> char* { return base ? base + off : reinterpret_cast<char*>((uintptr_t)off); };

  P->fac_begin = ar.take(0);
  for (int l = 0; l < n; ++l) {
    TLayer& t = P->L[l];
    t.Uo = ar.take((size_t)t.O * t.ro * 4);
    t.Ui = ar.take((size_t)t.I * t.ri * 4);
  }
  P->fac_end = ar.off;
  std::vector<OpGeom> og(4 * n);
  for (int l = 0; l < n; ++l) {
    TLayer& t = P->L[l];
    og[0 * n + l] = OpGeom(t.O, t.K2 * t.I, t.ro);
    og[1 * n + l] = OpGeom(t.O * t.K2, t.I, t.ri);
    og[2 * n + l] = OpGeom(t.O, t.K2 * t.ri, t.ro);
    og[3 * n + l] = OpGeom(t.ro * t.K2, t.I, t.ri);
    size_t xtb = 0, gpb = 0, vsb = 0, npad = 0;
    for (int k = 0; k < 4; ++k) {
      const OpGeom& g = og[k * n + l];
      t.reff[k] = g.r_eff;
      if (!jacobi_size_supported(g.N))
        CTX_FAIL(h, TADMM_ERR_UNSUPPORTED, "Tucker layer %d: eigen-problem of size %d exceeds the Jacobi kernels (max %d)", l, g.N, kJacobiMaxN);
      xtb = std::max(xtb, (size_t)g.Npad * g.ld * 8);
      gpb = std::max(gpb, (size_t)g.ksplit * (g.nt * (g.nt + 1) / 2) * 1024 * 8);
      vsb = std::max(vsb, (size_t)g.N * std::max(1, g.r_eff) * 4);
      npad = std::max<size_t>(npad, g.Npad);
    }
    t.T = ar.take((size_t)t.numel * 4);
    t.P = ar.take((size_t)std::max((int64_t)t.O * t.K2 * t.ri, (int64_t)t.ro * t.K2 * t.I) * 4);
    t.C = ar.take((size_t)t.ro * t.K2 * t.ri * 4);
    t.Vs = ar.take(vsb);
    t.XT = ar.take(xtb);
    t.gpart = ar.take(gpb);
    t.lam = ar.take(npad * 8);
    t.sigma = ar.take(npad * 8);
    t.order = ar.take(npad * 4);
    t.sblk = ar.take((npad / 16) * 256 * 8);
    t.bigG = 0;
    for (int k = 0; k < 2; ++k) {
      t.bigV[k] = 0;
      const int np = og[(2 + k) * n + l].Npad;
      t.warm[k] = jacobi_small_fits(np) ? ar.take((size_t)np * np * 8) : 0;
      const OpGeom& gk = og[(2 + k) * n + l];
      if (gk.ld > kLdResidentMax && warm_start_on()) {
        t.bigV[k] = ar.take((size_t)gk.Npad * gk.ld * 8);
        if (!t.bigG) t.bigG = ar.take(xtb);
      }
    }
  }
  P->off_off = ar.take((size_t)n * 3 * 8);
  P->done_off = ar.take((size_t)n * 4);
  P->prev_off = ar.take((size_t)n * 8);
  P->skip_off = ar.take((size_t)n * 4);
  P->warm_ok_off = ar.take((size_t)n * 2 * 4);
  P->nT_off = ar.take((size_t)n * 8);
  P->nC_off = ar.take((size_t)n * 8);
  P->err_off = ar.take((size_t)n * 2 * 8);
  P->iters_off = ar.take((size_t)n * 4);

  std::vector<SweepDesc> sd(n);
  std::vector<BlockRef> smap;
  for (int l = 0; l < n; ++l) {
    const TLayer& t = P->L[l];
    SweepDesc& s = sd[l];
    memset(&s, 0, sizeof s);
    s.W = W ? W[l] : nullptr; s.U = U ? U[l] : nullptr; s.Z = Z ? Z[l] : nullptr;
    s.T0 = (float*)dev(t.T);
    s.Zmat = (const float*)dev(t.T);
    s.O = t.O; s.I = t.I; s.K2 = t.K2;
    s.numel = t.numel;
    if (t.K2 > 1) {
      int ich = std::min(t.I, 256);
      while ((int64_t)t.K2 * (ich + 4) > 12288 && ich > 1) ich /= 2;
      s.ichunk = ich;
      s.nchunk = (t.I + ich - 1) / ich;
      s.nblk = t.O * s.nchunk;
    } else {
      s.ichunk = 8192;
      s.nchunk = (int)((t.numel + s.ichunk - 1) / s.ichunk);
      s.nblk = s.nchunk;
    }
    s.blk_begin = (int)smap.size();
    for (int b = 0; b < s.nblk; ++b) smap.push_back(BlockRef{l, b});
  }
  P->resid_partial_off = ar.take(smap.size() * 8);
  P->sweep_desc_off = da.take(sd.size() * sizeof(SweepDesc));
  if (img) img->put(P->sweep_desc_off, sd.data(), sd.size() * sizeof(SweepDesc));
  P->unfold.map_off = da.take(smap.size() * sizeof(BlockRef));
  P->unfold.nblocks = (int)smap.size();
  if (img) img->put(P->unfold.map_off, smap.data(), smap.size() * sizeof(BlockRef));
  P->fold = P->unfold;

  {
    std::vector<float> tol(n);
    std::vector<const float*> pT(n), pC(n);
    std::vector<int64_t> nT(n), nC(n);
    for (int l = 0; l < n; ++l) {
      const TLayer& t = P->L[l];
      tol[l] = P->descs[l].hooi_tol > 0.f ? P->descs[l].hooi_tol : 1e-4f;
      pT[l] = (const float*)dev(t.T); nT[l] = t.numel;
      pC[l] = (const float*)dev(t.C); nC[l] = (int64_t)t.ro * t.K2 * t.ri;
    }
    auto table = [&](const void* src, size_t bytes) {
      const size_t o = da.take(bytes);
      if (img) img->put(o, src, bytes);
      return o;
    };
    P->tol_off = table(tol.data(), (size_t)n * 4);
    P->ptrT_off = table(pT.data(), (size_t)n * 8);
    P->ptrC_off = table(pC.data(), (size_t)n * 8);
    P->numT_off = table(nT.data(), (size_t)n * 8);
    P->numC_off = table(nC.data(), (size_t)n * 8);
  }

  for (int k = 0; k < 4; ++k) {
    Lsv& v = P->lsv[k];
    const bool want_left = (k == 0 || k == 2);
    std::vector<GramDesc> gd(n);
    std::vector<EigDesc> ed(n);
    std::vector<GemmDesc> xg(n);
    std::vector<BlockRef> m_gp, m_gr, m_xg;
    std::vector<int> gp_cost(n);
    v.players_n.assign(n, 0);
    v.warm = false;
    v.big.clear();
    for (int l = 0; l < n; ++l) {
      const TLayer& t = P->L[l];
      const OpGeom& g = og[k * n + l];
      const float* A = (k < 2) ? (const float*)dev(t.T) : (const float*)dev(t.P);
      float* factor = want_left ? (float*)dev(t.Uo) : (float*)dev(t.Ui);
      const int r_full = want_left ? t.ro : t.ri;
      GramDesc& q = gd[l];
      memset(&q, 0, sizeof q);
      q.A = A; q.m = g.m; q.n = (int)g.cols; q.trans = g.trans ? 1 : 0; q.N = g.N; q.K = g.trans ? g.m : (int)g.cols;
      q.nt = g.nt; q.ksplit = g.ksplit; q.kchunk = g.kchunk;
      q.partial = (double*)dev(t.gpart); q.G = (double*)dev(t.XT); q.Npad = g.Npad; q.ld = g.ld;
      const int ntp = g.nt * (g.nt + 1) / 2;
      for (int b = 0; b < g.ksplit * ntp; ++b) m_gp.push_back(BlockRef{l, b});
      gp_cost[l] = g.kchunk;
      if (g.ksplit > 1)
        for (int b = 0; b < (int)(((int64_t)g.Npad * g.ld + 1023) / 1024); ++b) m_gr.push_back(BlockRef{l, b});
      const bool have_left = !g.trans;
      const bool direct = (have_left == want_left);
      EigDesc& e = ed[l];
      memset(&e, 0, sizeof e);
      e.XT = (double*)dev(t.XT); e.N = g.N; e.Npad = g.Npad; e.ld = g.ld; e.nb = g.nb;
      e.off = (double*)dev(P->off_off) + 3 * l;
      e.done = (int32_t*)dev(P->done_off) + l;
      e.lam = (double*)dev(t.lam); e.order = (int32_t*)dev(t.order); e.sigma = (double*)dev(t.sigma);
      e.r = g.r_eff; e.sblk = (double*)dev(t.sblk);
      if (k >= 2 && t.warm[k - 2] && warm_start_on()) {
        e.warm = (double*)dev(t.warm[k - 2]);
        e.warm_ok = (int32_t*)dev(P->warm_ok_off) + 2 * l + (k - 2);
        v.warm = true;
      }
      const bool big_apply = k >= 2 && t.bigV[k - 2];
      const bool big_save_only = k < 2 && t.bigV[k] && og[(k + 2) * n + l].N == g.N && og[(k + 2) * n + l].ld == g.ld;
      if (big_apply || big_save_only) {
        BigWarm bw;
        bw.layer = l; bw.Npad = g.Npad; bw.ld = g.ld; bw.apply = big_apply;
        bw.V = t.bigV[k & 1]; bw.Gt = t.bigG; bw.XT = t.XT;
        bw.ok = P->warm_ok_off + (size_t)(2 * l + (k & 1)) * 4;
        DgemmDesc dg;
        memset(&dg, 0, sizeof dg);
        dg.A = (const double*)dev(bw.V); dg.B = (const double*)dev(bw.Gt); dg.C = (const double*)dev(bw.XT);
        dg.selA = dg.selB = dg.selC = dg.selP = dg.selQ = -1;
        dg.M = dg.N = dg.K = g.Npad; dg.lda = dg.ldb = dg.ldc = g.ld;
        dg.tiles_m = g.Npad / 32; dg.tiles_n = g.Npad / 32;
        dg.gate = (const int32_t*)dev(bw.ok); dg.gate_min = 1;
        std::vector<BlockRef> m64;
        const int t64 = (g.Npad + 63) / 64;
        for (int b = 0; b < t64 * t64; ++b) m64.push_back(BlockRef{0, b});
        bw.nblocks = (int)m64.size();
        bw.desc_off = da.take(sizeof(DgemmDesc));
        bw.map_off = da.take(m64.size() * sizeof(BlockRef));
        if (img) img->put(bw.desc_off, &dg, sizeof dg);
        if (img) img->put(bw.map_off, m64.data(), m64.size() * sizeof(BlockRef));
        v.big.push_back(bw);
      }
      if (direct) { e.mode = 0; e.out_a = factor; e.ldo = r_full; }
      else { e.mode = 3; e.out_a = (float*)dev(t.Vs); e.ldo = 0; }
      v.players_n[l] = g.N;
      GemmDesc& x = xg[l];
      memset(&x, 0, sizeof x);
      if (!direct) {
        x.B = (const float*)dev(t.Vs); x.C = factor;
        x.N = g.r_eff; x.b_rs = g.r_eff; x.b_cs = 1; x.c_rs = r_full; x.c_cs = 1;
        x.alpha = 1.f; x.beta = 0.f;
        x.A = A;
        const int gn = (int)g.cols;
        if (want_left) { x.M = g.m; x.K = gn; x.a_rs = gn; x.a_cs = 1; }
        else { x.M = gn; x.K = g.m; x.a_rs = 1; x.a_cs = gn; }
        gemm_tiles(x, l, m_xg);
      }
    }
    std::stable_sort(m_gp.begin(), m_gp.end(),
                     [&](const BlockRef& a, const BlockRef& b) { return gp_cost[a.prob] > gp_cost[b.prob]; });
    place_phase(v.gram_p, da, img, gd.data(), gd.size() * sizeof(GramDesc), n, m_gp);
    place_map_like(v.gram_r, v.gram_p, da, img, m_gr);
    if (const int rc = build_eig_layout(h, v.eig, ed, false, da, img)) return rc;
    v.eig.prev_off = P->prev_off;
    place_phase(v.xg, da, img, xg.data(), xg.size() * sizeof(GemmDesc), n, m_xg);
  }

  for (int k = 0; k < 5; ++k) {
// ... 291 lines not shown
```

Before: 178.4 iters/s.

## Fold Jacobi convergence check into next sweep's first tick via packed tick records

```diff
diff --git a/dnn-compression-tensor-admm_amd/csrc/abi_ops.hip b/dnn-compression-tensor-admm_amd/csrc/abi_ops.hip
--- a/dnn-compression-tensor-admm_amd/csrc/abi_ops.hip
+++ b/dnn-compression-tensor-admm_amd/csrc/abi_ops.hip
@@ -436,17 +436,20 @@
   e.sblk = sblk;
   EigMaps maps;
   if (const int rc = eig_maps(h, L, ev, false, maps)) return rc;
-  const std::vector<BlockRef>* mv[3] = {&maps.tick, &maps.norm, &maps.ext};
+  const void* mv[3] = {maps.tick.data(), maps.norm.data(), maps.ext.data()};
+  const size_t mbytes[3] = {maps.tick.size() * sizeof(TickRec), maps.norm.size() * sizeof(BlockRef),
+                            maps.ext.size() * sizeof(BlockRef)};
+  if (mbytes[0] > (size_t)Npad * sizeof(BlockRef)) CTX_FAIL(h, TADMM_ERR_WORKSPACE, "internal: tick records exceed their slot");
   HIP_OK(h, hipMemcpyAsync(edev, &e, sizeof e, hipMemcpyHostToDevice, s));
   for (int i = 0; i < 3; ++i) {
     phases[i]->desc_off = o_desc;
     phases[i]->map_off = o_map[i];
-    HIP_OK(h, hipMemcpyAsync(base + o_map[i], mv[i]->data(), mv[i]->size() * sizeof(BlockRef), hipMemcpyHostToDevice, s));
+    HIP_OK(h, hipMemcpyAsync(base + o_map[i], mv[i], mbytes[i], hipMemcpyHostToDevice, s));
   }
   HIP_OK(h, hipStreamSynchronize(s));
   const bool super = L.kernel == EigTick::SuperPairs;
   const int units = L.players[0];
-  const BlockRef* m_tick = (const BlockRef*)(base + L.tick.map_off);
+  const TickRec* m_tick = (const TickRec*)(base + L.tick.map_off);
   const double tol = 1e-9;
   int tick = 0, gs = 0;
   bool conv = false;
@@ -473,7 +476,7 @@
   for (; gs < 40 && !conv; ++gs) {
     for (int t = 0; t < units - 1; ++t, ++tick) {
       if (super) {
-        HIP_OK(h, launch_jacobi_tick3(edev, m_tick, L.tick.nblocks, tick, tol, ld, s));
+        HIP_OK(h, launch_jacobi_tick3(m_tick, L.tick.nblocks, tick, tol, ld, s));
       } else {
         HIP_OK(h, launch_jacobi_tick(edev, m_tick, L.tick.nblocks, tick, tol, L.tick_lds, s));
       }
diff --git a/dnn-compression-tensor-admm_amd/csrc/common.h b/dnn-compression-tensor-admm_amd/csrc/common.h
--- a/dnn-compression-tensor-admm_amd/csrc/common.h
+++ b/dnn-compression-tensor-admm_amd/csrc/common.h
@@ -65,21 +65,41 @@
   double* scratch;
   int32_t period;
 };
+struct alignas(64) TickRec {
+  double* XT;
+  double* sblk;
+  double* off;
+  int32_t* done;
+  int32_t ld;
+  int32_t players;
+  int32_t period;
+  int32_t local;
+  int32_t prob;
+  int32_t pad[3];
+};
+static_assert(sizeof(TickRec) == 64, "a tick record is one 64-byte scalar load");
+
+struct TickRule {
+  double* hist = nullptr;
+  int32_t slot = 0;
+  int32_t* verdict = nullptr;
+};
 void launch_jacobi_init(const EigDesc* descs_dev, int nprob, hipStream_t s, const int32_t* skip = nullptr,
                         double* prev_dev = nullptr);
 void launch_jacobi_conv(const EigDesc* descs_dev, int nprob, int tick, double tol, bool super, double* prev_dev,
-                        int* verdict_pinned, hipStream_t s);
+                        int slot, int* verdict_pinned, hipStream_t s);
 constexpr int kJacobiMaxN = 8160;
 bool jacobi_size_supported(int n);
 size_t jacobi_tick_stream_lds_bytes();
 size_t jacobi_tick_lds_bytes(int ld_max);
-hipError_t launch_jacobi_tick(const EigDesc* descs_dev, const BlockRef* map_dev, int nblocks, int tick, double tol,
-                              size_t lds_bytes, hipStream_t s);
+bool jacobi_tick_streamed(size_t lds_bytes);
+hipError_t launch_jacobi_tick(const EigDesc* descs_dev, const TickRec* map_dev, int nblocks, int tick, double tol,
+                              size_t lds_bytes, hipStream_t s, const TickRule& rule = TickRule{});
 void dump_stamps();
 size_t jacobi_tick3_lds_bytes(int ld_max);
 bool jacobi_tick3_fits(int ld_max);
-hipError_t launch_jacobi_tick3(const EigDesc* descs_dev, const BlockRef* map_dev, int nblocks, int tick, double tol,
-                               int ld_max, hipStream_t s);
+hipError_t launch_jacobi_tick3(const TickRec* map_dev, int nblocks, int tick, double tol, int ld_max, hipStream_t s,
+                               const TickRule& rule = TickRule{});
 constexpr int kLdResidentMax = 1152;
 static inline int eig_ld(int N) { return (N + 127) / 128 * 128; }
 bool jacobi_small_fits(int npad_max);
diff --git a/dnn-compression-tensor-admm_amd/csrc/host.h b/dnn-compression-tensor-admm_amd/csrc/host.h
--- a/dnn-compression-tensor-admm_amd/csrc/host.h
+++ b/dnn-compression-tensor-admm_amd/csrc/host.h
@@ -88,15 +88,16 @@
   }
 };
 
+template <class Ref>
 static inline void place_phase(Phase& ph, Arena& da, HostImage* img, const void* descs, size_t dbytes, int nprob,
-                               const std::vector<BlockRef>& map) {
+                               const std::vector<Ref>& map) {
   ph.nprob = nprob;
   ph.nblocks = (int)map.size();
   ph.desc_off = da.take(std::max<size_t>(dbytes, 16));
-  ph.map_off = da.take(std::max<size_t>(map.size() * sizeof(BlockRef), 16));
+  ph.map_off = da.take(std::max<size_t>(map.size() * sizeof(Ref), 16));
   if (img) {
     img->put(ph.desc_off, descs, dbytes);
-    img->put(ph.map_off, map.data(), map.size() * sizeof(BlockRef));
+    img->put(ph.map_off, map.data(), map.size() * sizeof(Ref));
   }
 }
 
@@ -145,12 +146,13 @@
   return g;
 }
 
-static inline void xcd_group(std::vector<BlockRef>& m) {
+template <class Ref>
+static inline void xcd_group(std::vector<Ref>& m) {
   const char* e = getenv("TADMM_XCD_MAP");
   if (e && !atoi(e)) return;
   const int G = (int)m.size();
   if (G < 16) return;
-  std::vector<BlockRef> out(G);
+  std::vector<Ref> out(G);
   int i = 0;
   for (int x = 0; x < 8; ++x)
     for (int b = x; b < G; b += 8) out[b] = m[i++];
@@ -269,7 +271,7 @@
   EigTick kernel = EigTick::Pairs;
   int ld_max = 0;
   size_t tick_lds = 0;
-  const BlockRef* tick_map = nullptr; int tick_blocks = 0;
+  const TickRec* tick_map = nullptr; int tick_blocks = 0;
   double* prev_dev = nullptr;
   const int32_t* skip = nullptr;
   int npad_max = 0;
@@ -303,7 +305,7 @@
     g.players = players.data(); g.row_len = row_len.data(); g.mid_sizes = mid.data();
     g.gsteps = gsteps; g.kernel = kernel; g.aligned = aligned;
     g.ld_max = ld_max; g.npad_max = npad_max; g.tick_lds = tick_lds;
-    g.tick_map = (const BlockRef*)(ws + tick.map_off); g.tick_blocks = tick.nblocks;
+    g.tick_map = (const TickRec*)(ws + tick.map_off); g.tick_blocks = tick.nblocks;
     g.prev_dev = (double*)(ws + prev_off);
     g.skip = skip;
     return g;
@@ -319,7 +321,7 @@
   void finalize(char* ws, hipStream_t s, const int32_t* skip) const { sort(ws, s, skip); extract(ws, s, skip); }
 };
 
-struct EigMaps { std::vector<BlockRef> tick, norm, ext; };
+struct EigMaps { std::vector<TickRec> tick; std::vector<BlockRef> norm, ext; };
 static inline int eig_maps(tadmm_handle h, EigLayout& l, std::vector<EigDesc>& descs, bool align, EigMaps& m) {
   for (const EigDesc& e : descs)
     if (e.ld <= 0 || e.ld % 128)
@@ -339,13 +341,20 @@
     l.row_len.push_back(e.ld);
     l.mid.push_back((e.scratch && eig_mid_direct_size(e.N) && e.N == e.Npad) ? e.N : 0);
     l.gsteps = std::max(l.gsteps, units - 1);
-    for (int b = 0; b < units / 2; ++b) m.tick.push_back(BlockRef{pq, b});
     for (int b = 0; b < (e.Npad + 3) / 4; ++b) m.norm.push_back(BlockRef{pq, b});
     for (int b = 0; b < (e.r + 3) / 4; ++b) m.ext.push_back(BlockRef{pq, b});
   }
-  xcd_group(m.tick);
   l.aligned = super && align && align_sweeps_on();
   if (l.aligned) for (EigDesc& e : descs) e.period = l.gsteps;
+  for (int pq = 0; pq < l.neig; ++pq) {
+    const EigDesc& e = descs[pq];
+    TickRec t;
+    memset(&t, 0, sizeof t);
+    t.XT = e.XT; t.sblk = e.sblk; t.off = e.off; t.done = e.done;
+    t.ld = e.ld; t.players = l.players[pq]; t.period = super ? e.period : 0; t.prob = pq;
+    for (int b = 0; b < l.players[pq] / 2; ++b) { t.local = b; m.tick.push_back(t); }
+  }
+  xcd_group(m.tick);
   l.tick.nprob = l.norm.nprob = l.ext.nprob = l.neig;
   l.tick.nblocks = (int)m.tick.size();
   l.norm.nblocks = (int)m.norm.size(); l.ext.nblocks = (int)m.ext.size();
@@ -399,6 +408,7 @@
   bool all_done = false;
   int tick = 0, gs = 0, pending = -1, needed = 0;
   std::vector<char> known_done(g.neig, 0);
+  char carried[2] = {0, 0};
   if (super && g.mid_sizes && eig_mid_direct_on()) {
     bool any192 = false, any128 = false;
     for (int q = 0; q < g.neig; ++q) { any192 = any192 || g.mid_sizes[q] == 192; any128 = any128 || g.mid_sizes[q] == 128; }
@@ -427,17 +437,34 @@
     if (pending < 0) return TADMM_OK;
     if (hipEventSynchronize(poll.ev[pending & 1]) != hipSuccess) return TADMM_ERR_HIP;
     const int* v = poll.host + (size_t)(pending & 1) * poll.stride;
-    if (v[0]) { all_done = true; needed = pending + 1; }
+    bool all = v[0] != 0;
+    if (carried[pending & 1]) {
+      all = true;
+      for (int q = 0; q < g.neig; ++q) all = all && (v[1 + q] != 0 || g.players[q] < 2);
+    }
+    if (all) { all_done = true; needed = pending + 1; }
     for (int q = 0; q < g.neig; ++q) known_done[q] = v[1 + q] != 0;
     pending = -1;
     return TADMM_OK;
   };
+  static const bool lazy_poll = !(getenv("TADMM_POLL_EVERY_SWEEP") && atoi(getenv("TADMM_POLL_EVERY_SWEEP")));
+  static const bool tick_verdict = !(getenv("TADMM_TICK_VERDICT") && !atoi(getenv("TADMM_TICK_VERDICT")));
+  const bool can_defer = lazy_poll && tick_verdict && !(jt && jt->on) && !debug && g.prev_dev &&
+                         (super || !jacobi_tick_streamed(g.tick_lds));
+  int deferred = -1;
+  bool deferred_poll = false;
   for (; gs < max_sweeps && !all_done; ++gs) {
     for (int t = 0; t < g.gsteps; ++t, ++tick) {
+      TickRule rule;
+      const bool carries = t == 0 && deferred >= 0;
+      if (carries) {
+        rule.hist = g.prev_dev; rule.slot = deferred & 1;
+        if (deferred_poll) rule.verdict = poll.host + (size_t)(deferred & 1) * poll.stride;
+      }
       if (super) {
         const bool timed = jt && jt->on;
         if (timed) (void)hipEventRecord(jt->a, s);
-        HIP_OK(h, launch_jacobi_tick3(g.ed, g.tick_map, g.tick_blocks, tick, tol, g.ld_max, s));
+        HIP_OK(h, launch_jacobi_tick3(g.tick_map, g.tick_blocks, tick, tol, g.ld_max, s, rule));
         if (timed) {
           float ms = 0.f;
           (void)hipEventRecord(jt->b, s);
@@ -454,10 +481,20 @@
           }
         }
       } else {
-        HIP_OK(h, launch_jacobi_tick(g.ed, g.tick_map, g.tick_blocks, tick, tol, g.tick_lds, s));
-      }
-    }
-    launch_jacobi_conv(g.ed, g.neig, tick, tol, super, g.prev_dev, poll.host + (size_t)(gs & 1) * poll.stride, s);
+        HIP_OK(h, launch_jacobi_tick(g.ed, g.tick_map, g.tick_blocks, tick, tol, g.tick_lds, s, rule));
+      }
+      if (carries) {
+        if (deferred_poll) {
+          HIP_OK(h, hipEventRecord(poll.ev[deferred & 1], s));
+          pending = deferred;
+          carried[deferred & 1] = 1;
+        }
+        deferred = -1;
+      }
+    }
+    const bool defer = can_defer && g.expected > 0 && gs + 1 < g.expected && gs + 1 < max_sweeps;
+    if (!defer)
+      launch_jacobi_conv(g.ed, g.neig, tick, tol, super, g.prev_dev, gs, poll.host + (size_t)(gs & 1) * poll.stride, s);
     {
       const hipError_t le = hipGetLastError();
       if (le != hipSuccess) CTX_FAIL(h, TADMM_ERR_HIP, "Jacobi launch failed: %s", hipGetErrorString(le));
@@ -478,10 +515,11 @@
     int rc = consume();
     if (rc != TADMM_OK) CTX_FAIL(h, rc, "poll event failed");
     if (all_done) break;
-    static const bool lazy_poll = !(getenv("TADMM_POLL_EVERY_SWEEP") && atoi(getenv("TADMM_POLL_EVERY_SWEEP")));
+    if (defer) { deferred = gs; deferred_poll = gs + 3 >= g.expected; continue; }
     if (lazy_poll && !(jt && jt->on) && g.expected > 0 && gs + 3 < g.expected) continue;
     HIP_OK(h, hipEventRecord(poll.ev[gs & 1], s));
     pending = gs;
+    carried[gs & 1] = 0;
     if (g.expected > 0 && gs + 1 >= g.expected) {
       if (g.behind_last && behind_last_stands) { g.behind_last(s); stands = true; }
       rc = consume();
diff --git a/dnn-compression-tensor-admm_amd/csrc/jacobi.hip b/dnn-compression-tensor-admm_amd/csrc/jacobi.hip
--- a/dnn-compression-tensor-admm_amd/csrc/jacobi.hip
+++ b/dnn-compression-tensor-admm_amd/csrc/jacobi.hip
@@ -13,7 +13,7 @@
 __global__ __launch_bounds__(256) void jacobi_init_kernel(const EigDesc* __restrict__ descs,
                                                           const int32_t* __restrict__ skip, double* __restrict__ prev) {
   const EigDesc d = descs[blockIdx.x];
-  if (prev && threadIdx.x == 0) prev[blockIdx.x] = 0.0;
+  if (prev && threadIdx.x == 0) prev[2 * blockIdx.x] = prev[2 * blockIdx.x + 1] = 0.0;
   if (skip && skip[blockIdx.x]) {
     if (threadIdx.x == 0) *d.done = 1;
     return;
@@ -265,7 +265,7 @@
     sweep = tick / per;
     step = tick - sweep * per;
   }
-  __device__ __forceinline__ bool retired(const EigDesc& d, double tol, bool leader) const {
+  template <class D> __device__ __forceinline__ bool retired(const D& d, double tol, bool leader) const {
     if (*d.done) return true;
     if (step == 0 && sweep > 0 && d.off[(sweep - 1) & 1] < tol) {
       if (leader) *d.done = 1;
@@ -274,10 +274,10 @@
     return false;
   }
   struct State { int done; double prev, hmax; };
-  __device__ __forceinline__ State state(const EigDesc& d) const {
+  template <class D> __device__ __forceinline__ State state(const D& d) const {
     return State{*gp(d.done), gp(d.off)[(sweep - 1) & 1], gp(d.off)[2]};
   }
-  __device__ __forceinline__ bool retired(const EigDesc& d, const State& s, double tol, bool leader) const {
+  template <class D> __device__ __forceinline__ bool retired(const D& d, const State& s, double tol, bool leader) const {
     if (s.done) return true;
     if (step == 0 && sweep > 0 && s.prev < tol) {
       if (leader) *gp(d.done) = 1;
@@ -285,14 +285,45 @@
     }
     return false;
   }
-  __device__ __forceinline__ void record(const EigDesc& d, double mx) const {
+  __device__ __forceinline__ double history(const TickRule& r, int prob) const {
+    return r.hist ? gp(r.hist)[2 * prob + (r.slot ^ 1)] : 0.0;
+  }
+  template <class D>
+  __device__ __forceinline__ bool decide(const D& d, const State& s, double mp, const TickRule& r, int prob, double tol,
+                                         bool leader) const {
+    bool ret = retired(d, s, tol, leader);
+    if (!r.hist) return ret;
+    const bool own = step == 0 && sweep > 0;
+    if (!ret && own) {
+      const double m = s.prev;
+      if (mp > 0.0 && mp < 1e-1 && m < 1e-3) {
+        const double C = 10.0 * fmax(1.0, m / (mp * mp));
+        if (C * m * m < 10.0 * tol) {
+          ret = true;
+          if (leader) *gp(d.done) = 1;
+        }
+      }
+    }
+    if (leader) {
+      gp(r.hist)[2 * prob + r.slot] = (own && !s.done) ? s.prev : mp;
+      if (r.verdict) gp(r.verdict)[1 + prob] = ret ? 1 : 0;
+    }
+    return ret;
+  }
+  template <class D> __device__ __forceinline__ void record(const D& d, double mx) const {
     __hip_atomic_fetch_max(gp(reinterpret_cast<unsigned long long*>(&d.off[sweep & 1])),
                            (unsigned long long)__double_as_longlong(mx), __ATOMIC_RELAXED, __HIP_MEMORY_SCOPE_AGENT);
   }
-  __device__ __forceinline__ void clear_next(const EigDesc& d, bool leader) const {
+  template <class D> __device__ __forceinline__ void clear_next(const D& d, bool leader) const {
     if (step == steps - 1 && leader) gp(d.off)[(sweep + 1) & 1] = 0.0;
   }
 };
+
+__device__ __forceinline__ TickRec load_tick_rec(const TickRec* __restrict__ map) {
+  typedef int32_t rec_words_t __attribute__((ext_vector_type(16)));
+  const rec_words_t w = *(const G<rec_words_t>*)(map + blockIdx.x);
+  return __builtin_bit_cast(TickRec, w);
+}
 
 struct SlabCols {
   double* XT;
@@ -346,22 +377,23 @@
   }
 }
 
-__global__ __launch_bounds__(256) void jacobi_tick_kernel(const EigDesc* __restrict__ descs,
-                                                          const BlockRef* __restrict__ map, int tick, double tol) {
+__global__ __launch_bounds__(256) void jacobi_tick_kernel(const TickRec* __restrict__ map, int tick, double tol,
+                                                          TickRule rule) {
   extern __shared__ __attribute__((aligned(16))) double smem[];
-  const BlockRef br = map[blockIdx.x];
-  const EigDesc d = descs[br.prob];
-  const TickPos pos(tick, d.nb, 0);
+  const TickRec d = load_tick_rec(map);
+  const TickPos pos(tick, d.players, 0);
   const int tid = threadIdx.x, lane = tid & 63, wave = tid >> 6;
-  const bool leader = br.local == 0 && tid == 0;
-  const TickPos::State st = pos.state(d);
-  if (pos.retired(d, st, tol, leader)) return;
+  const bool leader = d.local == 0 && tid == 0;
+  TickPos::State st = pos.state(d);
+  double mp = pos.history(rule, d.prob);
+  asm volatile("" : "+s"(st.done), "+s"(st.prev), "+s"(st.hmax), "+s"(mp));
+  if (pos.decide(d, st, mp, rule, d.prob, tol, leader)) return;
   const int ld = d.ld, ldp = ld + 2;
   double* Xs = smem;
   const PairScratch S = carve_scratch(Xs + kPair * ldp);
 
   int ba, bb;
-  rr_pair(d.nb, pos.step, br.local, ba, bb);
+  rr_pair(d.players, pos.step, d.local, ba, bb);
   const int r = lane & 15, q = lane >> 4;
   const SlabCols cols{d.XT, ld, ba, bb, kJB, 0};
 
@@ -390,10 +422,10 @@
 constexpr int kStreamChunk = 1024;
 
 __global__ __launch_bounds__(256) void jacobi_tick_stream_kernel(const EigDesc* __restrict__ descs,
-                                                                 const BlockRef* __restrict__ map, int tick,
+                                                                 const TickRec* __restrict__ map, int tick,
                                                                  double tol) {
   extern __shared__ __attribute__((aligned(16))) double smem[];
-  const BlockRef br = map[blockIdx.x];
+  const BlockRef br{map[blockIdx.x].prob, map[blockIdx.x].local};
   const EigDesc d = descs[br.prob];
   const TickPos pos(tick, d.nb, 0);
   const int tid = threadIdx.x, lane = tid & 63, wave = tid >> 6;
@@ -496,22 +528,21 @@
   if (kLdsBarriers) lds_barrier(); else __syncthreads();
 }
 
-__global__ __launch_bounds__(512) void jacobi_tick3_kernel(const EigDesc* __restrict__ descs,
-                                                           const BlockRef* __restrict__ map, int tick, double tol) {
+__global__ __launch_bounds__(512) void jacobi_tick3_kernel(const TickRec* __restrict__ map, int tick, double tol,
+                                                           TickRule rule) {
   extern __shared__ __attribute__((aligned(16))) double smem[];
-  const BlockRef br = map[blockIdx.x];
-  const EigDesc d = descs[br.prob];
-  const TickPos pos(tick, d.nb >> 1, d.period);
+#ifdef TADMM_STAMPS
+  const unsigned long long t0 = clock64();
+  if (blockIdx.x == gridDim.x / 2 && threadIdx.x == 0) g_stamps[31] += 1;
+#endif
+  const TickRec d = load_tick_rec(map);
+  const TickPos pos(tick, d.players, d.period);
   if (pos.step >= pos.steps) return;
   const bool first = pos.step == 0;
   const int tid = threadIdx.x, lane = tid & 63, wave = tid >> 6;
   const int half = wave >> 2, wv = wave & 3, th = tid & 255;
-  const bool leader = br.local == 0 && tid == 0;
+  const bool leader = d.local == 0 && tid == 0;
   const int ld = d.ld, ldp = ld + 2;
-#ifdef TADMM_STAMPS
-  const unsigned long long t0 = clock64();
-  if (blockIdx.x == gridDim.x / 2 && tid == 0) g_stamps[31] += 1;
-#endif
   double* Xs = smem;
   double* R = Xs + kSuper * ldp;
   double (*H32)[kH32] = reinterpret_cast<double (*)[kH32]>(R);
@@ -524,16 +555,17 @@
   int* flags = reinterpret_cast<int*>(R + 2048 + 2 * (3 * kPair * kHP));
 
   int sa, sb;
-  rr_pair(d.nb >> 1, pos.step, br.local, sa, sb);
+  rr_pair(d.players, pos.step, d.local, sa, sb);
   const int r = lane & 15, q = lane >> 4;
   const SlabCols cols{d.XT, ld, sa, sb, kPair, 0};
   G<double>* sblk = gp(d.sblk) + (int64_t)(tid < 256 ? sa : sb) * (kPair * kPair) + th;
 
   dma_load_slab(Xs, ldp, cols, ld, wave, 8, lane);
   const TickPos::State st = pos.state(d);
+  const double mp = pos.history(rule, d.prob);
   double sreg = first ? 0.0 : *sblk;
   __builtin_amdgcn_s_waitcnt(0);
-  if (pos.retired(d, st, tol, leader)) return;
+  if (pos.decide(d, st, mp, rule, d.prob, tol, leader)) return;
   __syncthreads();
   STAMP(0, t0);
   pos.clear_next(d, leader);
@@ -906,7 +938,7 @@
 }
 
 __global__ __launch_bounds__(256) void jacobi_conv_kernel(const EigDesc* __restrict__ descs, int nprob, int tick,
-                                                          double tol, int super, double* __restrict__ prev,
+                                                          double tol, int super, double* prev, int slot,
                                                           int* __restrict__ verdict) {
   __shared__ int open_problems;
   if (threadIdx.x == 0) open_problems = 0;
@@ -917,17 +949,19 @@
     const int own = (super ? (d.nb >> 1) : d.nb) - 1;
     const int steps = (own > 0 && d.period > 0) ? d.period : own;
     bool conv = false;
+    const double mp = prev[2 * q + (slot ^ 1)];
+    double keep = mp;
     if (steps > 0 && tick % steps == 0) {
       const int swp = tick / steps - 1;
       const double m = d.off[swp & 1];
       conv = m < tol;
-      const double mp = prev[q];
       if (!conv && mp > 0.0 && mp < 1e-1 && m < 1e-3) {
         const double C = 10.0 * fmax(1.0, m / (mp * mp));
         conv = C * m * m < 10.0 * tol;
       }
-      prev[q] = m;
-    }
+      keep = m;
+    }
+    prev[2 * q + slot] = keep;
     if (conv) *d.done = 1;
     else open_problems = 1;
     verdict[1 + q] = conv ? 1 : 0;
@@ -937,10 +971,10 @@
 }
 
 void launch_jacobi_conv(const EigDesc* descs_dev, int nprob, int tick, double tol, bool super, double* prev_dev,
-                        int* verdict_pinned, hipStream_t s) {
+                        int slot, int* verdict_pinned, hipStream_t s) {
   if (nprob <= 0) return;
   hipLaunchKernelGGL(jacobi_conv_kernel, dim3(1), dim3(256), 0, s, descs_dev, nprob, tick, tol, super ? 1 : 0, prev_dev,
-                     verdict_pinned);
+                     slot & 1, verdict_pinned);
 }
 
 void launch_jacobi_init(const EigDesc* descs_dev, int nprob, hipStream_t s, const int32_t* skip, double* prev_dev) {
@@ -955,14 +989,14 @@
   return ((size_t)kSuper * (ld_max + 2) + 2048 + 2 * (3 * kPair * kHP)) * 8 + 32;
 }
 bool jacobi_tick3_fits(int ld_max) { return jacobi_tick3_lds_bytes(ld_max) <= 160 * 1024; }
-hipError_t launch_jacobi_tick3(const EigDesc* descs_dev, const BlockRef* map_dev, int nblocks, int tick, double tol,
-                               int ld_max, hipStream_t s) {
+hipError_t launch_jacobi_tick3(const TickRec* map_dev, int nblocks, int tick, double tol, int ld_max, hipStream_t s,
+                               const TickRule& rule) {
   if (nblocks <= 0) return hipSuccess;
   static DynLdsOptIn allow_lds;
   hipError_t e = allow_lds(jacobi_tick3_kernel, 160 * 1024);
   if (e != hipSuccess) return e;
-  hipLaunchKernelGGL(jacobi_tick3_kernel, dim3(nblocks), dim3(512), jacobi_tick3_lds_bytes(ld_max), s, descs_dev, map_dev,
-                     tick, tol);
+  hipLaunchKernelGGL(jacobi_tick3_kernel, dim3(nblocks), dim3(512), jacobi_tick3_lds_bytes(ld_max), s, map_dev, tick, tol,
+                     rule);
   e = hipPeekAtLastError();
   if (e != hipSuccess)
     fprintf(stderr, "[tadmm] jacobi tick3 launch failed: %s (blocks=%d lds=%zu)\n", hipGetErrorString(e), nblocks,
@@ -970,11 +1004,12 @@
   return hipSuccess;
 }
 
-hipError_t launch_jacobi_tick(const EigDesc* descs_dev, const BlockRef* map_dev, int nblocks, int tick, double tol,
-                              size_t lds_bytes, hipStream_t s) {
+bool jacobi_tick_streamed(size_t lds_bytes) { return lds_bytes > 160 * 1024; }
+hipError_t launch_jacobi_tick(const EigDesc* descs_dev, const TickRec* map_dev, int nblocks, int tick, double tol,
+                              size_t lds_bytes, hipStream_t s, const TickRule& rule) {
   if (nblocks <= 0) return hipSuccess;
   hipError_t e;
-  if (lds_bytes > 160 * 1024) {
+  if (jacobi_tick_streamed(lds_bytes)) {
     static DynLdsOptIn allow_lds;
     if ((e = allow_lds(jacobi_tick_stream_kernel, 160 * 1024)) != hipSuccess) return e;
     hipLaunchKernelGGL(jacobi_tick_stream_kernel, dim3(nblocks), dim3(256), jacobi_tick_stream_lds_bytes(), s, descs_dev,
@@ -982,7 +1017,7 @@
   } else {
     static DynLdsOptIn allow_tick_lds;
     if ((e = allow_tick_lds(jacobi_tick_kernel, 160 * 1024)) != hipSuccess) return e;
-    hipLaunchKernelGGL(jacobi_tick_kernel, dim3(nblocks), dim3(256), lds_bytes, s, descs_dev, map_dev, tick, tol);
+    hipLaunchKernelGGL(jacobi_tick_kernel, dim3(nblocks), dim3(256), lds_bytes, s, map_dev, tick, tol, rule);
   }
   e = hipPeekAtLastError();
   if (e != hipSuccess)
diff --git a/dnn-compression-tensor-admm_amd/csrc/plan.hip b/dnn-compression-tensor-admm_amd/csrc/plan.hip
--- a/dnn-compression-tensor-admm_amd/csrc/plan.hip
+++ b/dnn-compression-tensor-admm_amd/csrc/plan.hip
@@ -289,7 +289,7 @@
     sp.layer_of = layer_of;
     sp.off_off = ar.take((size_t)std::max(1, neig) * 3 * 8);
     sp.done_off = ar.take((size_t)std::max(1, neig) * 4);
-    sp.main.prev_off = ar.take((size_t)std::max(1, neig) * 8);
+    sp.main.prev_off = ar.take((size_t)std::max(1, neig) * 16);
     sp.skip_off = ar.take((size_t)std::max(1, neig) * 4);
     std::vector<FilterSpec> fspecs;
     sp.filt_of.clear();
@@ -411,7 +411,7 @@
       }
     }
     if (const int rc = build_eig_layout(h, sp.main, ed, true, da, img)) return rc;
-    sp.fb.prev_off = ar.take((size_t)std::max<size_t>(1, ed_fb.size()) * 8);
+    sp.fb.prev_off = ar.take((size_t)std::max<size_t>(1, ed_fb.size()) * 16);
     if (const int rc = build_eig_layout(h, sp.fb, ed_fb, true, da, img)) return rc;
     place_phase(sp.proj, da, img, pd.data(), pd.size() * sizeof(GemmDesc), neig, m_proj);
     sp.proj_repeatable = !pd.empty();
diff --git a/dnn-compression-tensor-admm_amd/csrc/tucker_plan.hip b/dnn-compression-tensor-admm_amd/csrc/tucker_plan.hip
--- a/dnn-compression-tensor-admm_amd/csrc/tucker_plan.hip
+++ b/dnn-compression-tensor-admm_amd/csrc/tucker_plan.hip
@@ -214,7 +214,7 @@
   }
   P->off_off = ar.take((size_t)n * 3 * 8);
   P->done_off = ar.take((size_t)n * 4);
-  P->prev_off = ar.take((size_t)n * 8);
+  P->prev_off = ar.take((size_t)n * 16);
   P->skip_off = ar.take((size_t)n * 4);
   P->warm_ok_off = ar.take((size_t)n * 2 * 4);
   P->nT_off = ar.take((size_t)n * 8);
```

Result: no change. 179.8 iters/s, median of 6 (+0.8%).
